# Cc19245/gaussian-splatting_CC-Comments

Hardware: AMD Instinct MI355X
Metric: train iters/sec (fwd+bwd rasterize) @1980x1080, 1M Gaussians (higher is better)
Workload: dtype f32; 1 GPU; C3: 1000000 Gaussians, SH deg 3, 1980x1080, mu=-5.0, seed 0; P=1000000, parallelism=single view

## Files before the change

gaussian-splatting_cc-comments_amd/csrc/api.hip:

```cpp
#include <stdarg.h>
#include <stdio.h>
#include <string.h>

#include <atomic>
#include <mutex>
#include <string>
#include <vector>

#include "gsr_internal.h"
#include "../../include/gsr_aa.h"

#define GSR_MAX_DEVICES 64
#ifndef GSR_COLOR_BESIDE_WGS
#define GSR_COLOR_BESIDE_WGS 2
#endif
#define GSR_COLOR_BESIDE_MAX_P 1500000

static thread_local char g_err[512] = "";

int gsr_fail(int code, const char* fmt, ...)
{
	va_list ap;
	va_start(ap, fmt);
	vsnprintf(g_err, sizeof g_err, fmt, ap);
	va_end(ap);
	return code;
}

int gsr_check_hip(hipError_t e, const char* what)
{
	if (e == hipSuccess) return GSR_OK;
	return gsr_fail(GSR_ERR_HIP, "%s: %s", what, hipGetErrorString(e));
}

int gsr_stage_done(hipStream_t s, int debug, const char* stage)
{
	hipError_t e = hipGetLastError();
	if (e != hipSuccess) return gsr_fail(GSR_ERR_HIP, "launch of %s failed: %s", stage, hipGetErrorString(e));
	if (debug & GSR_DEBUG_SYNC) {
		e = hipStreamSynchronize(s);
		if (e != hipSuccess) return gsr_fail(GSR_ERR_HIP, "[HIP ERROR] in stage %s: %s", stage, hipGetErrorString(e));
	}
	return GSR_OK;
}

extern "C" const char* gsr_last_error(void) { return g_err; }
extern "C" const char* gsr_version(void) { return "gsr-hip gfx950 r4"; }

struct ProfEntry { const char* name; hipEvent_t a, b; };
struct ProfRecorder {
	hipStream_t stream;
	bool on = false, open = false;
	std::vector<ProfEntry> ev;
	size_t used = 0;
	char only[64] = "";
};
static std::mutex g_prof_mu;
static std::vector<ProfRecorder*> g_prof;
static std::atomic<int> g_prof_active{0};

static ProfRecorder* prof_find(hipStream_t s, bool create)
{
	for (ProfRecorder* r : g_prof)
		if (r->stream == s) return r;
	if (!create) return nullptr;
	ProfRecorder* r = new ProfRecorder();
	r->stream = s;
	g_prof.push_back(r);
	return r;
}

static ProfEntry& prof_next(ProfRecorder* r, const char* name)
{
	if (r->used == r->ev.size()) {
		ProfEntry e;
		e.name = name;
		(void)hipEventCreate(&e.a);
		(void)hipEventCreate(&e.b);
		r->ev.push_back(e);
	}
	ProfEntry& e = r->ev[r->used++];
	e.name = name;
	return e;
}

bool gsr_prof_kernel_events(hipStream_t s, const char* name, hipEvent_t* a, hipEvent_t* b)
{
	if (g_prof_active.load(std::memory_order_relaxed) == 0) return false;
	std::lock_guard<std::mutex> lk(g_prof_mu);
	ProfRecorder* r = prof_find(s, false);
	if (!r || !r->on || !r->only[0] || strcmp(r->only, name) != 0) return false;
	ProfEntry& e = prof_next(r, name);
	r->open = false;
	*a = e.a;
	*b = e.b;
	return true;
}

void gsr_prof_mark_begin(hipStream_t s, const char* name)
{
	if (!name || g_prof_active.load(std::memory_order_relaxed) == 0) return;
	std::lock_guard<std::mutex> lk(g_prof_mu);
	ProfRecorder* r = prof_find(s, false);
	if (!r || !r->on) return;
	r->open = false;
	if (r->only[0] && strcmp(r->only, name) != 0) return;
	r->open = true;
	(void)hipEventRecord(prof_next(r, name).a, s);
}

void gsr_prof_mark_end(hipStream_t s)
{
	if (g_prof_active.load(std::memory_order_relaxed) == 0) return;
	std::lock_guard<std::mutex> lk(g_prof_mu);
	ProfRecorder* r = prof_find(s, false);
	if (!r || !r->on || !r->open || r->used == 0) return;
	r->open = false;
	(void)hipEventRecord(r->ev[r->used - 1].b, s);
}

static bool gsr_prof_records_all(hipStream_t s)
{
	if (g_prof_active.load(std::memory_order_relaxed) == 0) return false;
	std::lock_guard<std::mutex> lk(g_prof_mu);
	ProfRecorder* r = prof_find(s, false);
	return r && r->on && !r->only[0];
}

extern "C" int gsr_profile_begin_only(void* stream, const char* stage)
{
	std::lock_guard<std::mutex> lk(g_prof_mu);
	ProfRecorder* r = prof_find((hipStream_t)stream, true);
	if (!r->on) g_prof_active.fetch_add(1);
	r->on = true;
	r->open = false;
	r->used = 0;
	r->only[0] = 0;
	if (stage) { strncpy(r->only, stage, sizeof r->only - 1); r->only[sizeof r->only - 1] = 0; }
	return GSR_OK;
}

extern "C" int gsr_profile_begin(void* stream) { return gsr_profile_begin_only(stream, nullptr); }

extern "C" int gsr_profile_end(void* stream, gsr_kernel_time* out, int capacity)
{
	std::lock_guard<std::mutex> lk(g_prof_mu);
	ProfRecorder* r = prof_find((hipStream_t)stream, false);
	if (!r || !r->on) return 0;
	r->on = false;
	g_prof_active.fetch_sub(1);
	int n = 0;
	for (size_t k = 0; k < r->used; k++) {
		ProfEntry& e = r->ev[k];
		(void)hipEventSynchronize(e.b);
		float ms = 0.f;
		(void)hipEventElapsedTime(&ms, e.a, e.b);
		if (out && n < capacity) { out[n].name = e.name; out[n].ms = ms; n++; }
	}
	r->used = 0;
	return n;
}

extern "C" int gsr_geometry_layout_of(int P, gsr_geometry_layout* o)
{
	if (P < 0 || !o) return gsr_fail(GSR_ERR_INVALID_ARGUMENT, "gsr_geometry_layout_of: bad arguments");
	const size_t n = (size_t)P;
	const size_t nb = (n + GSR_PREPROCESS_BLOCK - 1) / GSR_PREPROCESS_BLOCK;
	size_t off = 0;
	o->splat = off;          off = gsr_align_up(off + n * sizeof(GsrSplat));
	o->depth_keys = off;     off = gsr_align_up(off + n * 4);
	o->depth_keys_alt = off; off = gsr_align_up(off + n * 4);
	o->perm = off;           off = gsr_align_up(off + n * 4);
	o->perm_alt = off;       off = gsr_align_up(off + n * 4);
	o->tiles_touched = off;  off = gsr_align_up(off + n * 4);
	o->rect = off;           off = gsr_align_up(off + n * 8);
	o->slot_base = off;      off = gsr_align_up(off + n * 4);
	o->clamped = off;        off = gsr_align_up(off + n);
	o->sh_ddir = off;        off = gsr_align_up(off + n * 36);
	o->status = off;         off = gsr_align_up(off + GSR_STATUS_WORDS * 4);
	o->scan_temp = off;      off = gsr_align_up(off + 2 * gsr_align_up(nb * 4));
	o->sort_table = off;     off = gsr_align_up(off + gsr_radix_table_bytes(n));
	o->col_table = off;      off = gsr_align_up(off + gsr_tilebin_col_table_bytes(n));
	o->rshape = off;         off = gsr_align_up(off + n * 8);
	o->total = off;
	return GSR_OK;
}

extern "C" int gsr_image_layout_of(int W, int H, gsr_image_layout* o)
{
	if (W < 0 || H < 0 || !o) return gsr_fail(GSR_ERR_INVALID_ARGUMENT, "gsr_image_layout_of: bad arguments");
	const size_t N = (size_t)W * H, T = (size_t)gsr_grid_x(W) * gsr_grid_y(H);
	size_t off = 0;
	o->final_C = off;          off = gsr_align_up(off + 3 * N * 4);
	o->final_T = off;          off = gsr_align_up(off + N * 4);
	o->n_contrib = off;        off = gsr_align_up(off + N * 4);
	o->ranges = off;           off = gsr_align_up(off + T * 8);
	o->tile_max_contrib = off; off = gsr_align_up(off + T * 4);
	{
		const size_t extra_f = 3 * (size_t)gsr_tile_order_max_split((int)T), extra_b = gsr_tile_order_max_segments((int)T);
		o->tile_order = off;   off = gsr_align_up(off + (T + (extra_f > extra_b ? extra_f : extra_b) + 1) * 4);
	}
	o->total = off;
	return GSR_OK;
}

extern "C" int gsr_binning_layout_of(int P, int64_t R, int W, int H, gsr_binning_layout* o)
{
	(void)P;
	if (R < 0 || W < 0 || H < 0 || !o) return gsr_fail(GSR_ERR_INVALID_ARGUMENT, "gsr_binning_layout_of: bad arguments");
	const size_t n = (size_t)R;
	size_t off = 0;
	o->point_list = off;     off = gsr_align_up(off + n * 4);
	o->point_list_alt = off; off = gsr_align_up(off + n * 4);
	o->tile_keys = off;      off = gsr_align_up(off + n * 4);
	o->tile_keys_alt = off;  off = gsr_align_up(off + n * 4);
	{
		const size_t a = gsr_radix_table_bytes(n), b = gsr_tilebin_row_table_bytes(n);
		o->sort_table = off; off = gsr_align_up(off + (a > b ? a : b));
	}
	o->checkpoints = off;    off = gsr_align_up(off + gsr_checkpoint_records(R) * 256 * sizeof(float4));
	o->total = off;
	o->tile_key_bytes = (size_t)gsr_tile_key_bytes(gsr_grid_x(W) * gsr_grid_y(H), n);
	o->column_pairs = gsr_tilebin_applies(W, H) ? 1 : 0;
	return GSR_OK;
}

extern "C" size_t gsr_geometry_bytes(int P)
{
	gsr_geometry_layout l;
	return gsr_geometry_layout_of(P, &l) == GSR_OK ? l.total : 0;
}
extern "C" size_t gsr_image_bytes(int W, int H)
{
	gsr_image_layout l;
	return gsr_image_layout_of(W, H, &l) == GSR_OK ? l.total : 0;
}
extern "C" size_t gsr_binning_bytes(int P, int64_t R, int W, int H)
{
	gsr_binning_layout l;
	return gsr_binning_layout_of(P, R, W, H, &l) == GSR_OK ? l.total : 0;
}
extern "C" size_t gsr_backward_scratch_bytes(int P, int64_t R)
{
	(void)P;
	if (R < 0) return 0;
	return gsr_align_up((size_t)R * sizeof(GsrGradSlot));
}

extern "C" int gsr_aux_layout_of(int64_t R, int W, int H, gsr_aux_layout* o)
{
	if (R < 0 || W < 0 || H < 0 || !o) return gsr_fail(GSR_ERR_INVALID_ARGUMENT, "gsr_aux_layout_of: bad arguments");
	size_t off = 0;
	o->ckpt_depth = off; off = gsr_align_up(off + gsr_checkpoint_records(R) * 256 * sizeof(float));
	o->final_D = off;    off = gsr_align_up(off + (size_t)W * H * sizeof(float));
	o->total = off;
	return GSR_OK;
}
extern "C" size_t gsr_aux_bytes(int64_t R, int W, int H)
{
	gsr_aux_layout l;
	return gsr_aux_layout_of(R, W, H, &l) == GSR_OK ? l.total : 0;
}
static const GsrAuxBlend* gsr_aux_view(const gsr_aux_args* x, int64_t R, int W, int H, GsrAuxBlend* a)
{
	if (!x) return nullptr;
	gsr_aux_layout l;
	gsr_aux_layout_of(R, W, H, &l);
	char* b = (char*)x->scratch;
	a->out_depth = x->out_depth; a->out_alpha = x->out_alpha;
	a->ckpt_depth = (float*)(b + l.ckpt_depth);
	a->final_D = (float*)(b + l.final_D);
	a->dL_ddepth = x->dL_ddepth; a->dL_dalpha = x->dL_dalpha;
	return a;
}

static bool aligned16(const void* p) { return ((uintptr_t)p & 15u) == 0; }

enum GsrAuxNeeds {
	GSR_AUX_NEEDS_MODE,
	GSR_AUX_NEEDS_SCRATCH,
	GSR_AUX_NEEDS_OUTPUTS
};
static int gsr_option_check(const char* who, int antialiasing, const gsr_aux_args* aux, bool optional, GsrAuxNeeds needs, bool live)
{
	if (antialiasing != 0 && antialiasing != 1) return gsr_fail(GSR_ERR_INVALID_ARGUMENT, "%s: antialiasing must be 0 or 1, got %d", who, antialiasing);
	if (!aux) return optional ? GSR_OK : gsr_fail(GSR_ERR_INVALID_ARGUMENT, "%s: aux is NULL", who);
	if (aux->mode != GSR_AUX_DEPTH && aux->mode != GSR_AUX_INVDEPTH) return gsr_fail(GSR_ERR_INVALID_ARGUMENT, "%s: the mode of aux is unknown", who);
	if (needs == GSR_AUX_NEEDS_MODE) return GSR_OK;
	if (!aligned16(aux->scratch)) return gsr_fail(GSR_ERR_INVALID_ARGUMENT, "%s: scratch must be 16-byte aligned", who);
	if (live && (!aux->scratch || (needs == GSR_AUX_NEEDS_OUTPUTS && (!aux->out_depth || !aux->out_alpha))))
		return gsr_fail(GSR_ERR_INVALID_ARGUMENT, "%s: %sscratch is NULL", who, needs == GSR_AUX_NEEDS_OUTPUTS ? "out_depth, out_alpha or " : "");
	return GSR_OK;
}

GsrGeometry gsr_geometry_view(void* blob, int P)
{
	gsr_geometry_layout l;
	gsr_geometry_layout_of(P, &l);
	char* b = (char*)blob;
	GsrGeometry g;
	g.splat = (GsrSplat*)(b + l.splat);
	g.depth_keys = (uint32_t*)(b + l.depth_keys);
	g.depth_keys_alt = (uint32_t*)(b + l.depth_keys_alt);
	g.perm = (uint32_t*)(b + l.perm);
	g.perm_alt = (uint32_t*)(b + l.perm_alt);
	g.tiles_touched = (uint32_t*)(b + l.tiles_touched);
	g.rect = (uint2*)(b + l.rect);
	g.slot_base = (uint32_t*)(b + l.slot_base);
	g.clamped = (uint8_t*)(b + l.clamped);
	g.sh_ddir = (float*)(b + l.sh_ddir);
	g.status = (uint32_t*)(b + l.status);
	g.sorted_block_sums = (uint32_t*)(b + l.scan_temp);
	g.block_tiles = (uint32_t*)(b + l.scan_temp + gsr_align_up(((size_t)P + GSR_PREPROCESS_BLOCK - 1) / GSR_PREPROCESS_BLOCK * 4));
	g.sort_table = (void*)(b + l.sort_table);
	g.col_table = (void*)(b + l.col_table);
	g.rshape = (uint2*)(b + l.rshape);
	return g;
}

GsrImage gsr_image_view(void* blob, int W, int H)
{
	gsr_image_layout l;
	gsr_image_layout_of(W, H, &l);
	char* b = (char*)blob;
	GsrImage im;
	im.final_C = (float*)(b + l.final_C);
	im.final_T = (float*)(b + l.final_T);
	im.n_contrib = (uint32_t*)(b + l.n_contrib);
	im.ranges = (uint2*)(b + l.ranges);
	im.tile_max_contrib = (uint32_t*)(b + l.tile_max_contrib);
	im.tile_order = (uint32_t*)(b + l.tile_order);
	return im;
}

GsrBinning gsr_binning_view(void* blob, int P, int64_t R, int W, int H)
{
	gsr_binning_layout l;
	gsr_binning_layout_of(P, R, W, H, &l);
	char* b = (char*)blob;
	GsrBinning bn;
	bn.point_list = (uint32_t*)(b + l.point_list);
	bn.point_list_alt = (uint32_t*)(b + l.point_list_alt);
	bn.tile_keys = (uint32_t*)(b + l.tile_keys);
	bn.tile_keys_alt = (uint32_t*)(b + l.tile_keys_alt);
	bn.sort_table = (void*)(b + l.sort_table);
	bn.checkpoints = (float4*)(b + l.checkpoints);
	return bn;
}

extern "C" uint32_t gsr_get_higher_msb(uint32_t n)
{
	uint32_t msb = sizeof(n) * 4;
	uint32_t step = msb;
	while (step > 1) {
		step /= 2;
		if (n >> msb) msb += step; else msb -= step;
	}
	if (n >> msb) msb++;
	return msb;
}

struct GsrThreadDevice {
	hipStream_t aux_stream = nullptr;
	hipEvent_t aux_fork = nullptr, aux_join = nullptr;
	uint32_t* status_host = nullptr;
	hipEvent_t status_event = nullptr;
	hipStream_t copy_stream = nullptr;
	hipEvent_t copy_fork = nullptr;
};
struct GsrThreadState { GsrThreadDevice dev[GSR_MAX_DEVICES]; };
static thread_local GsrThreadState g_thread;

extern "C" int gsr_thread_release(void)
{
	g_err[0] = 0;
	int rc = GSR_OK;
	for (int d = 0; d < GSR_MAX_DEVICES; d++) {
		GsrThreadDevice& t = g_thread.dev[d];
		if (t.aux_stream) { (void)hipStreamSynchronize(t.aux_stream); if (hipStreamDestroy(t.aux_stream) != hipSuccess) rc = GSR_ERR_HIP; }
		if (t.aux_fork && hipEventDestroy(t.aux_fork) != hipSuccess) rc = GSR_ERR_HIP;
		if (t.aux_join && hipEventDestroy(t.aux_join) != hipSuccess) rc = GSR_ERR_HIP;
		if (t.status_event && hipEventDestroy(t.status_event) != hipSuccess) rc = GSR_ERR_HIP;
		if (t.copy_stream) { (void)hipStreamSynchronize(t.copy_stream); if (hipStreamDestroy(t.copy_stream) != hipSuccess) rc = GSR_ERR_HIP; }
		if (t.copy_fork && hipEventDestroy(t.copy_fork) != hipSuccess) rc = GSR_ERR_HIP;
		if (t.status_host && hipHostFree(t.status_host) != hipSuccess) rc = GSR_ERR_HIP;
		t = GsrThreadDevice();
	}
	if (rc) { (void)hipGetLastError(); return gsr_fail(rc, "gsr_thread_release: a HIP resource could not be freed"); }
	return GSR_OK;
}

static bool gsr_helper_stream(hipStream_t* stream, hipEvent_t* e0, hipEvent_t* e1)
{
	if (*stream) return true;
	hipStream_t st = nullptr;
	hipEvent_t a = nullptr, b = nullptr;
	if (hipStreamCreateWithFlags(&st, hipStreamNonBlocking) == hipSuccess && hipEventCreateWithFlags(&a, hipEventDisableTiming) == hipSuccess &&
	    (!e1 || hipEventCreateWithFlags(&b, hipEventDisableTiming) == hipSuccess)) {
		*stream = st; *e0 = a;
		if (e1) *e1 = b;
		return true;
	}
	(void)hipGetLastError();
	if (st) (void)hipStreamDestroy(st);
	if (a) (void)hipEventDestroy(a);
	if (b) (void)hipEventDestroy(b);
	return false;
}

struct GsrJoinOnExit {
	hipStream_t s;
	hipEvent_t ev = nullptr;
	explicit GsrJoinOnExit(hipStream_t st) : s(st) {}
	void arm(hipEvent_t e) { ev = e; }
	int now()
	{
		if (!ev) return GSR_OK;
		hipEvent_t e = ev;
		ev = nullptr;
		if (hipStreamWaitEvent(s, e, 0) == hipSuccess) return GSR_OK;
		(void)hipEventSynchronize(e);
		return gsr_fail(GSR_ERR_HIP, "hipStreamWaitEvent(join) failed");
	}
	~GsrJoinOnExit()
	{
		if (ev && hipStreamWaitEvent(s, ev, 0) != hipSuccess) (void)hipEventSynchronize(ev);
	}
};

struct GsrDrainOnExit {
	hipStream_t st = nullptr;
	void arm(hipStream_t s) { st = s; }
	void disarm() { st = nullptr; }
	~GsrDrainOnExit() { if (st) (void)hipStreamSynchronize(st); }
};

struct GsrLastStage1 { const void* geometry = nullptr; bool col_pairs = false; };
static thread_local GsrLastStage1 g_last_stage1;

static int gsr_forward_preprocess_impl(const GsrPreprocessArgs& in, void* geometry, int64_t* num_rendered_host, void* stream, int debug,
                                       int aux, int aa)
{
	g_err[0] = 0;
	hipStream_t s = (hipStream_t)stream;
	GsrPreprocessArgs a = in;
	const int P = a.P, width = a.W, height = a.H;
	if (!num_rendered_host) return gsr_fail(GSR_ERR_INVALID_ARGUMENT, "num_rendered_host is NULL");
	*num_rendered_host = 0;
	if (P < 0 || width <= 0 || height <= 0) return gsr_fail(GSR_ERR_INVALID_ARGUMENT, "bad P / image size");
	if (P == 0) return GSR_OK;
	if (!a.means3D || !a.opacities || !a.viewmatrix || !a.projmatrix || !geometry)
		return gsr_fail(GSR_ERR_INVALID_ARGUMENT, "gsr_forward_preprocess: required pointer is NULL");
	if (!a.colors_precomp && !a.shs)
		return gsr_fail(GSR_ERR_INVALID_ARGUMENT, "For non-RGB, provide precomputed Gaussian colors!");
	if (!a.colors_precomp && (a.M <= 0 || (a.D + 1) * (a.D + 1) > a.M || a.D < 0 || a.D > 3 || !a.cam_pos))
		return gsr_fail(GSR_ERR_INVALID_ARGUMENT, "SH degree %d needs %d coefficients, M = %d", a.D, (a.D + 1) * (a.D + 1), a.M);
	if (!a.cov3D_precomp && (!a.scales || !a.rotations))
		return gsr_fail(GSR_ERR_INVALID_ARGUMENT, "provide scales+rotations or cov3D_precomp");
	if (width > 65535 * GSR_TILE_X || height > 65535 * GSR_TILE_Y)
		return gsr_fail(GSR_ERR_INVALID_ARGUMENT, "image too large for 16-bit tile coordinates");
	if (!aligned16(geometry)) return gsr_fail(GSR_ERR_INVALID_ARGUMENT, "geometry buffer must be 16-byte aligned");

	if (a.leaf && (a.M > 1 && !a.shs_rest)) return gsr_fail(GSR_ERR_INVALID_ARGUMENT, "leaf mode: features_rest is NULL");
	if (a.leaf && a.M > 16) return gsr_fail(GSR_ERR_INVALID_ARGUMENT, "leaf mode: at most 16 SH coefficients (degree 3), M = %d", a.M);
	a.focal_y = height / (2.0f * a.tan_fovy);
	a.focal_x = width / (2.0f * a.tan_fovx);
	a.g = gsr_geometry_view(geometry, P);

	int rc;
	int device = 0;
	if ((rc = gsr_check_hip(hipGetDevice(&device), "hipGetDevice"))) return rc;
	if (device < 0 || device >= GSR_MAX_DEVICES) return gsr_fail(GSR_ERR_INVALID_ARGUMENT, "device index %d not supported", device);
	GsrThreadDevice& td = g_thread.dev[device];
	const bool col_pairs = gsr_tilebin_applies(width, height) && !(debug & GSR_DEBUG_TILE_SORT);
	a.trim = (col_pairs && !(debug & GSR_DEBUG_NO_TRIM)) ? 1 : 0;
	const bool color = gsr_preprocess_needs_color(a);
#ifdef GSR_AB_FORCE_RADIX_DEPTH
	const bool bucket = false;
#else
	const bool bucket = gsr_bucket_sort_applies(P) && !(debug & GSR_DEBUG_RADIX_DEPTH);
#endif
	const bool beside = color && !(debug & (GSR_DEBUG_SYNC | GSR_DEBUG_SERIAL)) && !gsr_prof_records_all(s) &&
	                    gsr_helper_stream(&td.aux_stream, &td.aux_fork, &td.aux_join);
	GsrJoinOnExit join(s);
	gsr_launch_zero_status(a.g.status, s, beside ? td.aux_fork : nullptr);
	if (beside) {
		if ((rc = gsr_check_hip(hipStreamWaitEvent(td.aux_stream, td.aux_fork, 0), "hipStreamWaitEvent(fork)"))) return rc;
		gsr_launch_preprocess_color(a, td.aux_stream, P <= GSR_COLOR_BESIDE_MAX_P ? GSR_COLOR_BESIDE_WGS : 0, aux);
		if (hipEventRecord(td.aux_join, td.aux_stream) != hipSuccess) {
			(void)hipStreamSynchronize(td.aux_stream);
			return gsr_fail(GSR_ERR_HIP, "hipEventRecord(join) failed");
		}
		join.arm(td.aux_join);
	}
	const bool copy_beside = !(debug & (GSR_DEBUG_SYNC | GSR_DEBUG_SERIAL)) && !gsr_prof_records_all(s) &&
	                         gsr_helper_stream(&td.copy_stream, &td.copy_fork, nullptr);
	{
		GsrProfScope p(s, "preprocess");
		gsr_launch_preprocess(a, s, copy_beside ? td.copy_fork : nullptr, aux, aa);
	}
	if ((rc = gsr_stage_done(s, debug, "preprocess"))) return rc;
	if (color && !beside) {
		GsrProfScope p(s, "preprocess_color");
		gsr_launch_preprocess_color(a, s, 0, aux);
	}
	if ((rc = gsr_stage_done(s, debug, "preprocess_color"))) return rc;

	if (!td.status_host) {
		if ((rc = gsr_check_hip(hipHostMalloc((void**)&td.status_host, GSR_STATUS_WORDS * 4, hipHostMallocDefault), "hipHostMalloc"))) return rc;
	}
	if (!td.status_event) {
		if ((rc = gsr_check_hip(hipEventCreateWithFlags(&td.status_event, hipEventDisableTiming), "hipEventCreate"))) return rc;
	}
	uint32_t* status_host = td.status_host;
	hipEvent_t ev = td.status_event;
	if (copy_beside && (rc = gsr_check_hip(hipStreamWaitEvent(td.copy_stream, td.copy_fork, 0), "hipStreamWaitEvent(copy fork)"))) return rc;
	hipStream_t cs = copy_beside ? td.copy_stream : s;
	GsrDrainOnExit drain;
	if (copy_beside) drain.arm(td.copy_stream);
	if ((rc = gsr_check_hip(hipMemcpyAsync(status_host, a.g.status, GSR_STATUS_WORDS * 4, hipMemcpyDeviceToHost, cs), "hipMemcpyAsync(num_rendered)"))) return rc;
	if ((rc = gsr_check_hip(hipEventRecord(ev, cs), "hipEventRecord"))) return rc;
	const uint32_t* bias = a.g.status + GSR_STATUS_NEGMIN;
	{
		GsrProfScope p(s, "depth_sort");
		if (bucket) {
			gsr_launch_depth_bucket_sort(a.g, P, col_pairs ? gsr_tilebin_seg(a.g, P) : nullptr, s);
			if (col_pairs) gsr_launch_tilebin_col_hist(a.g, P, 0, s, true);
			else gsr_launch_sorted_block_sums(a.g, P, 0, s);
		} else {
			gsr_radix_sort_passes(a.g.depth_keys, a.g.perm, a.g.depth_keys_alt, a.g.perm_alt, (size_t)P, 32, 4, 0, 3, a.g.sort_table, bias, 4, s);
			if (col_pairs) gsr_launch_tilebin_col_hist(a.g, P, 1, s);
			else gsr_launch_sorted_block_sums(a.g, P, 1, s);
			gsr_launch_slot_base_finish(a.g.slot_base, a.g.block_tiles, a.g.status, (size_t)P, s);
		}
	}
	if ((rc = gsr_stage_done(s, debug, "depth_sort"))) return rc;
	if ((rc = gsr_check_hip(hipEventSynchronize(ev), "hipEventSynchronize(num_rendered)"))) return rc;
	drain.disarm();
	g_last_stage1.geometry = geometry;
	g_last_stage1.col_pairs = col_pairs;
	if (status_host[0] & 1u)
		return gsr_fail(GSR_ERR_PREFILTERED, "Point is filtered although prefiltered is set. This shouldn't happen!");
	int64_t total = 0;
	uint32_t negmin = 0, kmax = 0;
	for (int k = 0; k < GSR_COUNT_PARTS; k++) {
		total += (int64_t)status_host[4 + k];
		negmin = status_host[GSR_STATUS_NEGMIN + k] > negmin ? status_host[GSR_STATUS_NEGMIN + k] : negmin;
		kmax = status_host[GSR_STATUS_MAX + k] > kmax ? status_host[GSR_STATUS_MAX + k] : kmax;
	}
	*num_rendered_host = total;
	const uint32_t kmin = ~negmin;
	const uint32_t culled_value = kmax >= kmin ? (kmax - kmin) + 1u : 0u;
	const int fourth = !bucket && ((culled_value >> 24) != 0u || (kmax >= kmin && kmax - kmin == 0xFFFFFFFFu));
	if ((rc = join.now())) return rc;
	if (fourth) {
		GsrProfScope p(s, "depth_sort");
		gsr_radix_sort_passes(a.g.depth_keys, a.g.perm, a.g.depth_keys_alt, a.g.perm_alt, (size_t)P, 32, 4, 3, 1, a.g.sort_table, bias, 4, s);
		if (col_pairs) {
			if ((rc = gsr_check_hip(hipMemsetAsync(a.g.col_table, 0, gsr_tilebin_col_clear_words((size_t)P) * 4, s), "hipMemsetAsync(col_table)"))) return rc;
			gsr_launch_tilebin_col_hist(a.g, P, 0, s);
		} else {
			gsr_launch_sorted_block_sums(a.g, P, 0, s);
		}
	}
	return gsr_stage_done(s, debug, "depth_sort");
}

static GsrPreprocessArgs gsr_preprocess_inputs(int P, int D, int M, int width, int height, const float* means3D, const float* shs,
                                               const float* colors_precomp, const float* opacities, const float* scales,
                                               float scale_modifier, const float* rotations, const float* cov3D_precomp,
                                               const float* viewmatrix, const float* projmatrix, const float* cam_pos, float tan_fovx,
                                               float tan_fovy, int prefiltered, int* radii)
{
	GsrPreprocessArgs a = {};
	a.P = P; a.D = D; a.M = M; a.W = width; a.H = height;
	a.means3D = means3D; a.shs = shs; a.colors_precomp = colors_precomp; a.opacities = opacities;
	a.scales = scales; a.scale_modifier = scale_modifier; a.rotations = rotations; a.cov3D_precomp = cov3D_precomp;
	a.viewmatrix = viewmatrix; a.projmatrix = projmatrix; a.cam_pos = cam_pos;
	a.tan_fovx = tan_fovx; a.tan_fovy = tan_fovy;
	a.prefiltered = prefiltered;
	a.radii = radii;
	return a;
}
static GsrPreprocessArgs gsr_preprocess_leaves(int P, int D, int M, int width, int height, const float* xyz, const float* features_dc,
                                               const float* features_rest, const float* opacity_logits, const float* log_scales,
                                               float scale_modifier, const float* raw_rotations, const float* viewmatrix,
                                               const float* projmatrix, const float* cam_pos, float tan_fovx, float tan_fovy,
                                               int prefiltered, int* radii)
{
	GsrPreprocessArgs a = gsr_preprocess_inputs(P, D, M, width, height, xyz, features_dc, nullptr, opacity_logits, log_scales, scale_modifier,
	                                            raw_rotations, nullptr, viewmatrix, projmatrix, cam_pos, tan_fovx, tan_fovy, prefiltered, radii);
	a.leaf = 1; a.shs_rest = features_rest;
	return a;
}

extern "C" int gsr_forward_preprocess(int P, int D, int M, int width, int height, const float* means3D,
                                      const float* shs, const float* colors_precomp, const float* opacities,
                                      const float* scales, float scale_modifier, const float* rotations,
                                      const float* cov3D_precomp, const float* viewmatrix, const float* projmatrix,
                                      const float* cam_pos, float tan_fovx, float tan_fovy, int prefiltered,
                                      int* radii, void* geometry, int64_t* num_rendered_host, void* stream, int debug)
{
	const GsrPreprocessArgs a = gsr_preprocess_inputs(P, D, M, width, height, means3D, shs, colors_precomp, opacities, scales, scale_modifier, rotations,
	                                                    cov3D_precomp, viewmatrix, projmatrix, cam_pos, tan_fovx, tan_fovy, prefiltered, radii);
	return gsr_forward_preprocess_impl(a, geometry, num_rendered_host, stream, debug, 0, 0);
}

extern "C" int gsr_forward_preprocess_leaf(int P, int D, int M, int width, int height, const float* xyz,
                                           const float* features_dc, const float* features_rest,
                                           const float* opacity_logits, const float* log_scales, float scale_modifier,
                                           const float* raw_rotations, const float* viewmatrix, const float* projmatrix,
                                           const float* cam_pos, float tan_fovx, float tan_fovy, int prefiltered,
                                           int* radii, void* geometry, int64_t* num_rendered_host, void* stream,
                                           int debug)
{
	const GsrPreprocessArgs a = gsr_preprocess_leaves(P, D, M, width, height, xyz, features_dc, features_rest, opacity_logits, log_scales, scale_modifier,
	                                                    raw_rotations, viewmatrix, projmatrix, cam_pos, tan_fovx, tan_fovy, prefiltered, radii);
	return gsr_forward_preprocess_impl(a, geometry, num_rendered_host, stream, debug, 0, 0);
}

extern "C" int gsr_forward_preprocess_aux(const gsr_aux_args* aux, int P, int D, int M, int width, int height, const float* means3D,
                                          const float* shs, const float* colors_precomp, const float* opacities,
                                          const float* scales, float scale_modifier, const float* rotations,
                                          const float* cov3D_precomp, const float* viewmatrix, const float* projmatrix,
                                          const float* cam_pos, float tan_fovx, float tan_fovy, int prefiltered,
                                          int* radii, void* geometry, int64_t* num_rendered_host, void* stream, int debug)
{
	int rc;
	if ((rc = gsr_option_check("gsr_forward_preprocess_aux", 0, aux, false, GSR_AUX_NEEDS_MODE, false))) return rc;
	const GsrPreprocessArgs a = gsr_preprocess_inputs(P, D, M, width, height, means3D, shs, colors_precomp, opacities, scales, scale_modifier, rotations,
	                                                    cov3D_precomp, viewmatrix, projmatrix, cam_pos, tan_fovx, tan_fovy, prefiltered, radii);
	return gsr_forward_preprocess_impl(a, geometry, num_rendered_host, stream, debug, aux->mode, 0);
}

extern "C" int gsr_forward_preprocess_leaf_aux(const gsr_aux_args* aux, int P, int D, int M, int width, int height, const float* xyz,
                                               const float* features_dc, const float* features_rest,
                                               const float* opacity_logits, const float* log_scales, float scale_modifier,
                                               const float* raw_rotations, const float* viewmatrix, const float* projmatrix,
                                               const float* cam_pos, float tan_fovx, float tan_fovy, int prefiltered,
                                               int* radii, void* geometry, int64_t* num_rendered_host, void* stream,
                                               int debug)
{
	int rc;
	if ((rc = gsr_option_check("gsr_forward_preprocess_leaf_aux", 0, aux, false, GSR_AUX_NEEDS_MODE, false))) return rc;
	const GsrPreprocessArgs a = gsr_preprocess_leaves(P, D, M, width, height, xyz, features_dc, features_rest, opacity_logits, log_scales, scale_modifier,
	                                                    raw_rotations, viewmatrix, projmatrix, cam_pos, tan_fovx, tan_fovy, prefiltered, radii);
	return gsr_forward_preprocess_impl(a, geometry, num_rendered_host, stream, debug, aux->mode, 0);
}

extern "C" int gsr_forward_preprocess_aa(int antialiasing, const gsr_aux_args* aux, int P, int D, int M, int width, int height,
                                         const float* means3D, const float* shs, const float* colors_precomp, const float* opacities,
                                         const float* scales, float scale_modifier, const float* rotations,
                                         const float* cov3D_precomp, const float* viewmatrix, const float* projmatrix,
                                         const float* cam_pos, float tan_fovx, float tan_fovy, int prefiltered,
                                         int* radii, void* geometry, int64_t* num_rendered_host, void* stream, int debug)
{
	int rc;
	if ((rc = gsr_option_check("gsr_forward_preprocess_aa", antialiasing, aux, true, GSR_AUX_NEEDS_MODE, false))) return rc;
	const GsrPreprocessArgs a = gsr_preprocess_inputs(P, D, M, width, height, means3D, shs, colors_precomp, opacities, scales, scale_modifier, rotations,
	                                                    cov3D_precomp, viewmatrix, projmatrix, cam_pos, tan_fovx, tan_fovy, prefiltered, radii);
	return gsr_forward_preprocess_impl(a, geometry, num_rendered_host, stream, debug, aux ? aux->mode : 0, antialiasing);
}

extern "C" int gsr_forward_preprocess_leaf_aa(int antialiasing, const gsr_aux_args* aux, int P, int D, int M, int width, int height,
                                              const float* xyz, const float* features_dc, const float* features_rest,
                                              const float* opacity_logits, const float* log_scales, float scale_modifier,
                                              const float* raw_rotations, const float* viewmatrix, const float* projmatrix,
                                              const float* cam_pos, float tan_fovx, float tan_fovy, int prefiltered,
                                              int* radii, void* geometry, int64_t* num_rendered_host, void* stream,
                                              int debug)
{
	int rc;
	if ((rc = gsr_option_check("gsr_forward_preprocess_leaf_aa", antialiasing, aux, true, GSR_AUX_NEEDS_MODE, false))) return rc;
	const GsrPreprocessArgs a = gsr_preprocess_leaves(P, D, M, width, height, xyz, features_dc, features_rest, opacity_logits, log_scales, scale_modifier,
	                                                    raw_rotations, viewmatrix, projmatrix, cam_pos, tan_fovx, tan_fovy, prefiltered, radii);
	return gsr_forward_preprocess_impl(a, geometry, num_rendered_host, stream, debug, aux ? aux->mode : 0, antialiasing);
}

static int gsr_forward_render_impl(int P, int64_t R, int width, int height, const float* background,
                                   const int* radii, void* geometry, void* binning, void* image, float* out_color,
                                   void* stream, int debug, const gsr_aux_args* aux)
{
	g_err[0] = 0;
	hipStream_t s = (hipStream_t)stream;
	if (P < 0 || R < 0 || width <= 0 || height <= 0) return gsr_fail(GSR_ERR_INVALID_ARGUMENT, "bad sizes");
	if (P == 0) return GSR_OK;
	if (!background || !geometry || !image || !out_color || (R > 0 && !binning))
		return gsr_fail(GSR_ERR_INVALID_ARGUMENT, "gsr_forward_render: required pointer is NULL");
	if (!aligned16(geometry) || !aligned16(image) || !aligned16(binning))
		return gsr_fail(GSR_ERR_INVALID_ARGUMENT, "state buffers must be 16-byte aligned");
	if (R > 0xffffffffLL) return gsr_fail(GSR_ERR_INVALID_ARGUMENT, "num_rendered exceeds 32-bit offsets");
	if ((int64_t)gsr_grid_x(width) * gsr_grid_y(height) >= (1 << 28))
		return gsr_fail(GSR_ERR_INVALID_ARGUMENT, "image too large: more than 2^28 tiles");

	GsrGeometry g = gsr_geometry_view(geometry, P);
	GsrImage im = gsr_image_view(image, width, height);
	const int ntiles = gsr_grid_x(width) * gsr_grid_y(height);
	int rc;
	int key_bytes = 4;
	GsrBinning b;
	memset(&b, 0, sizeof b);
	const bool col_pairs = gsr_tilebin_applies(width, height) && !(debug & GSR_DEBUG_TILE_SORT);
	if (g_last_stage1.geometry == geometry && g_last_stage1.col_pairs != col_pairs)
		return gsr_fail(GSR_ERR_INVALID_ARGUMENT, "gsr_forward_render: GSR_DEBUG_TILE_SORT must be passed to both forward calls or to neither "
		                "(gsr_forward_preprocess on this thread prepared this geometry buffer for the other binning)");
	if (R > 0) b = gsr_binning_view(binning, P, R, width, height);
	if (R > 0 && col_pairs) {
		{
			GsrProfScope p(s, "col_scatter");
			gsr_launch_tilebin_col_scatter(g, P, b, R, s);
		}
		if ((rc = gsr_stage_done(s, debug, "col_scatter"))) return rc;
		{
			GsrProfScope p(s, "row_hist");
			gsr_launch_tilebin_row_hist(g, P, b, R, s);
		}
		if ((rc = gsr_stage_done(s, debug, "row_hist"))) return rc;
		{
			GsrProfScope p(s, "row_scatter");
			gsr_launch_tilebin_row_scatter(g, P, b, R, im.ranges, width, height, s);
		}
		if ((rc = gsr_stage_done(s, debug, "row_scatter"))) return rc;
	} else {
		if (R > 0) {
			const int bit = (int)gsr_get_higher_msb((uint32_t)ntiles);
			const bool even = gsr_radix_num_passes(bit) % 2 == 0;
			uint32_t *k0 = even ? b.tile_keys : b.tile_keys_alt, *v0 = even ? b.point_list : b.point_list_alt;
			uint32_t *k1 = even ? b.tile_keys_alt : b.tile_keys, *v1 = even ? b.point_list_alt : b.point_list;
			key_bytes = gsr_tile_key_bytes(ntiles, (size_t)R);
			{
				GsrProfScope p(s, "duplicate_keys");
				gsr_launch_duplicate_keys(g, P, width, k0, key_bytes, v0, (uint32_t*)b.sort_table, gsr_radix_clear_words((size_t)R), s);
			}
			if ((rc = gsr_stage_done(s, debug, "duplicate_keys"))) return rc;
			{
				GsrProfScope p(s, "sort");
				int in_first = 1;
				gsr_radix_sort_u32(k0, v0, k1, v1, (size_t)R, bit, b.sort_table, &in_first, 0, key_bytes, s);
			}
			if ((rc = gsr_stage_done(s, debug, "sort"))) return rc;
		}
		{
			GsrProfScope p(s, "tile_ranges");
			gsr_launch_tile_ranges(b.tile_keys, key_bytes, R, im.ranges, ntiles, b.tile_keys_alt, s);
		}
		if ((rc = gsr_stage_done(s, debug, "tile_ranges"))) return rc;
	}
	if (R > 0) {
		GsrProfScope p(s, "tile_order");
		gsr_launch_tile_order(im, ntiles, false, R, !(debug & GSR_DEBUG_NO_SPLIT), s, col_pairs);
	}
	if ((rc = gsr_stage_done(s, debug, "tile_order"))) return rc;
	{
		GsrProfScope p(s, "render_forward");
		GsrAuxBlend x;
		gsr_launch_render_forward(width, height, im, b.point_list, g.splat, b.checkpoints, background, out_color, R > 0, !(debug & GSR_DEBUG_NO_CULL), s,
		                          gsr_aux_view(aux, R, width, height, &x));
	}
	return gsr_stage_done(s, debug, "render_forward");
}

extern "C" int gsr_forward_render(int P, int64_t R, int width, int height, const float* background,
                                  const int* radii, void* geometry, void* binning, void* image, float* out_color,
                                  void* stream, int debug)
{
	return gsr_forward_render_impl(P, R, width, height, background, radii, geometry, binning, image, out_color, stream, debug, nullptr);
}

extern "C" int gsr_forward_render_aux(const gsr_aux_args* aux, int P, int64_t R, int width, int height, const float* background,
                                      const int* radii, void* geometry, void* binning, void* image, float* out_color,
                                      void* stream, int debug)
{
	int rc;
	if ((rc = gsr_option_check("gsr_forward_render_aux", 0, aux, false, GSR_AUX_NEEDS_OUTPUTS, P > 0))) return rc;
	return gsr_forward_render_impl(P, R, width, height, background, radii, geometry, binning, image, out_color, stream, debug, aux);
}

static int gsr_backward_check(const gsr_backward_args& a, const char* who)
{
	if (a.P < 0 || a.num_rendered < 0 || a.width <= 0 || a.height <= 0) return gsr_fail(GSR_ERR_INVALID_ARGUMENT, "%s: bad sizes", who);
	if (a.P == 0) return GSR_OK;
	if (!a.background || !a.means3D || !a.viewmatrix || !a.projmatrix || !a.geometry || !a.image || !a.dL_dpix ||
	    !a.dL_dmean2D || !a.dL_dopacity || !a.dL_dmean3D || !a.dL_dscale || !a.dL_drot || (a.num_rendered > 0 && (!a.binning || !a.scratch)))
		return gsr_fail(GSR_ERR_INVALID_ARGUMENT, "gsr_backward: required pointer is NULL");
	if (!a.leaf && ((a.colors_precomp && !a.dL_dcolor) || (a.cov3D_precomp && !a.dL_dcov3D) || (a.shs && !a.dL_dsh && !a.dL_dcolor)))
		return gsr_fail(GSR_ERR_INVALID_ARGUMENT, "gsr_backward: the gradient of a provided input is NULL");
	if (a.leaf) {
		if (!a.shs || !a.scales || !a.rotations || (a.M > 1 && !a.shs_rest))
			return gsr_fail(GSR_ERR_INVALID_ARGUMENT, "gsr_backward_leaf: a leaf tensor is NULL");
		if (a.M > 16) return gsr_fail(GSR_ERR_INVALID_ARGUMENT, "gsr_backward_leaf: at most 16 SH coefficients (degree 3), M = %d", a.M);
		if ((a.dL_dsh == nullptr) != (a.dL_dsh_rest == nullptr) && a.M > 1)
			return gsr_fail(GSR_ERR_INVALID_ARGUMENT, "gsr_backward_leaf: pass both feature gradients or neither");
		if (!a.dL_dsh && !a.dL_dcolor)
			return gsr_fail(GSR_ERR_INVALID_ARGUMENT, "gsr_backward_leaf: without feature gradients dL_dRGB is required");
	}
	if (a.stat_max_radii2D && !a.radii)
		return gsr_fail(GSR_ERR_INVALID_ARGUMENT, "gsr_backward: stat_max_radii2D needs radii");
	if (!aligned16(a.geometry) || !aligned16(a.image) || !aligned16(a.binning) || !aligned16(a.scratch))
		return gsr_fail(GSR_ERR_INVALID_ARGUMENT, "state buffers must be 16-byte aligned");
	return GSR_OK;
}

static uint8_t* gsr_slot_valid_of(const gsr_backward_args& a)
{
	if (a.num_rendered <= 0) return nullptr;
	return (uint8_t*)gsr_binning_view(a.binning, a.P, a.num_rendered, a.width, a.height).tile_keys_alt;
}

static int gsr_backward_blend_impl(const gsr_backward_args* args, const gsr_aux_args* aux)
{
	g_err[0] = 0;
	if (!args) return gsr_fail(GSR_ERR_INVALID_ARGUMENT, "gsr_backward_blend: args is NULL");
	const gsr_backward_args& a = *args;
	int rc;
	if ((rc = gsr_backward_check(a, "gsr_backward_blend"))) return rc;
	if (a.P == 0 || a.num_rendered == 0) return GSR_OK;
	hipStream_t s = (hipStream_t)a.stream;
	GsrGeometry g = gsr_geometry_view(a.geometry, a.P);
	GsrImage im = gsr_image_view(a.image, a.width, a.height);
	GsrBinning b = gsr_binning_view(a.binning, a.P, a.num_rendered, a.width, a.height);
	{
		GsrProfScope p(s, "tile_order");
		gsr_launch_tile_order(im, gsr_grid_x(a.width) * gsr_grid_y(a.height), true, a.num_rendered, !(a.debug & GSR_DEBUG_NO_SPLIT), s);
	}
	if ((rc = gsr_stage_done(s, a.debug, "tile_order"))) return rc;
	{
		hipEvent_t t0 = nullptr, t1 = nullptr;
		const bool own = gsr_prof_kernel_events(s, "render_backward", &t0, &t1);
		GsrProfScope p(s, own ? nullptr : "render_backward");
		GsrAuxBlend x;
		gsr_launch_render_backward(a.width, a.height, im, b.point_list, g.splat, b.checkpoints, g.slot_base, a.background, a.dL_dpix,
		                           (GsrGradSlot*)a.scratch, (uint8_t*)b.tile_keys_alt, !(a.debug & GSR_DEBUG_NO_CULL), s, t0, t1,
		                           gsr_aux_view(aux, a.num_rendered, a.width, a.height, &x));
	}
	return gsr_stage_done(s, a.debug, "render_backward");
}

extern "C" int gsr_backward_blend(const gsr_backward_args* args) { return gsr_backward_blend_impl(args, nullptr); }

extern "C" int gsr_backward_blend_aux(const gsr_backward_args* args, const gsr_aux_args* aux)
{
	int rc;
	if ((rc = gsr_option_check("gsr_backward_blend_aux", 0, aux, false, GSR_AUX_NEEDS_SCRATCH, args && args->P > 0 && args->num_rendered > 0))) return rc;
	return gsr_backward_blend_impl(args, aux);
}

static int gsr_backward_gaussians_impl(const gsr_backward_args* args, int first, int count, int out_row0, int aux, const float* aa_opacities)
{
	g_err[0] = 0;
	if (!args) return gsr_fail(GSR_ERR_INVALID_ARGUMENT, "gsr_backward_gaussians: args is NULL");
	const gsr_backward_args& b = *args;
	int rc;
	if ((rc = gsr_backward_check(b, "gsr_backward_gaussians"))) return rc;
	if (first < 0 || count < 0 || (int64_t)first + count > b.P || (first & 63) || (out_row0 != 0 && out_row0 != first))
		return gsr_fail(GSR_ERR_INVALID_ARGUMENT, "gsr_backward_gaussians: bad range [%d, %d + %d) of %d Gaussians (first must be a multiple "
		                "of 64, out_row0 must be 0 or first)", first, first, count, b.P);
	if (count == 0) return GSR_OK;
	hipStream_t s = (hipStream_t)b.stream;
	GsrGaussianBackwardArgs a = {};
	a.leaf = b.leaf; a.shs_rest = b.shs_rest; a.dL_dsh_rest = b.dL_dsh_rest;
	a.P = b.P; a.D = b.D; a.M = b.M; a.W = b.width; a.H = b.height;
	a.first = first; a.count = count; a.out_row0 = out_row0;
	a.means3D = b.means3D; a.shs = b.shs; a.colors_precomp = b.colors_precomp; a.scales = b.scales;
	a.scale_modifier = b.scale_modifier; a.rotations = b.rotations; a.cov3D_precomp = b.cov3D_precomp;
	a.viewmatrix = b.viewmatrix; a.projmatrix = b.projmatrix; a.cam_pos = b.cam_pos;
	a.tan_fovx = b.tan_fovx; a.tan_fovy = b.tan_fovy;
	a.focal_y = b.height / (2.0f * b.tan_fovy);
	a.focal_x = b.width / (2.0f * b.tan_fovx);
	a.radii = b.radii; a.g = gsr_geometry_view(b.geometry, b.P);
	a.slots = (const GsrGradSlot*)b.scratch; a.slot_valid = gsr_slot_valid_of(b);
	a.dL_dmean2D = b.dL_dmean2D; a.dL_dconic = b.dL_dconic; a.dL_dopacity = b.dL_dopacity; a.dL_dcolor = b.dL_dcolor;
	a.dL_dmean3D = b.dL_dmean3D; a.dL_dcov3D = b.dL_dcov3D; a.dL_dsh = b.dL_dsh; a.dL_dscale = b.dL_dscale; a.dL_drot = b.dL_drot;
	a.stat_xyz_gradient_accum = b.stat_xyz_gradient_accum; a.stat_denom = b.stat_denom; a.stat_max_radii2D = b.stat_max_radii2D;
	{
		GsrProfScope p(s, "gaussian_backward");
		gsr_launch_gaussian_backward(a, aa_opacities, s, aux);
	}
	return gsr_stage_done(s, b.debug, "gaussian_backward");
}

extern "C" int gsr_backward_gaussians(const gsr_backward_args* args, int first, int count, int out_row0)
{
	return gsr_backward_gaussians_impl(args, first, count, out_row0, 0, nullptr);
}

extern "C" int gsr_backward_gaussians_aux(const gsr_backward_args* args, const gsr_aux_args* aux, int first, int count, int out_row0)
{
	int rc;
	if ((rc = gsr_option_check("gsr_backward_gaussians_aux", 0, aux, false, GSR_AUX_NEEDS_SCRATCH, false))) return rc;
	return gsr_backward_gaussians_impl(args, first, count, out_row0, aux->mode, nullptr);
}

extern "C" int gsr_backward_gaussians_aa(const gsr_backward_args* args, int antialiasing, const float* opacities, const gsr_aux_args* aux,
                                         int first, int count, int out_row0)
{
	int rc;
	if ((rc = gsr_option_check("gsr_backward_gaussians_aa", antialiasing, aux, true, GSR_AUX_NEEDS_SCRATCH, false))) return rc;
	if (antialiasing && args && args->P > 0 && count > 0 && !opacities)
		return gsr_fail(GSR_ERR_INVALID_ARGUMENT, "gsr_backward_gaussians_aa: the opacity input is NULL");
	return gsr_backward_gaussians_impl(args, first, count, out_row0, aux ? aux->mode : 0, antialiasing ? opacities : nullptr);
}

static int gsr_backward_whole(const gsr_backward_args& a)
{
	int rc;
	if ((rc = gsr_backward_blend(&a))) return rc;
	return gsr_backward_gaussians(&a, 0, a.P, 0);
}

extern "C" int gsr_backward(int P, int D, int M, int64_t R, int width, int height, const float* background,
                            const float* means3D, const float* shs, const float* colors_precomp,
                            const float* scales, float scale_modifier, const float* rotations,
                            const float* cov3D_precomp, const float* viewmatrix, const float* projmatrix,
                            const float* cam_pos, float tan_fovx, float tan_fovy, const int* radii, void* geometry,
                            void* binning, void* image, void* scratch, const float* dL_dpix, float* dL_dmean2D,
                            float* dL_dconic, float* dL_dopacity, float* dL_dcolor, float* dL_dmean3D,
                            float* dL_dcov3D, float* dL_dsh, float* dL_dscale, float* dL_drot, void* stream,
                            int debug)
{
	gsr_backward_args a = {};
	a.P = P; a.D = D; a.M = M; a.num_rendered = R; a.width = width; a.height = height; a.leaf = 0;
	a.background = background; a.means3D = means3D; a.shs = shs; a.colors_precomp = colors_precomp; a.scales = scales;
	a.scale_modifier = scale_modifier; a.rotations = rotations; a.cov3D_precomp = cov3D_precomp; a.viewmatrix = viewmatrix;
	a.projmatrix = projmatrix; a.cam_pos = cam_pos; a.tan_fovx = tan_fovx; a.tan_fovy = tan_fovy; a.radii = radii;
	a.geometry = geometry; a.binning = binning; a.image = image; a.scratch = scratch; a.dL_dpix = dL_dpix;
	a.dL_dmean2D = dL_dmean2D; a.dL_dconic = dL_dconic; a.dL_dopacity = dL_dopacity; a.dL_dcolor = dL_dcolor;
	a.dL_dmean3D = dL_dmean3D; a.dL_dcov3D = dL_dcov3D; a.dL_dsh = dL_dsh; a.dL_dscale = dL_dscale; a.dL_drot = dL_drot;
	a.stream = stream; a.debug = debug;
	return gsr_backward_whole(a);
}

extern "C" int gsr_backward_leaf(int P, int D, int M, int64_t R, int width, int height, const float* background,
                                 const float* xyz, const float* features_dc, const float* features_rest,
                                 const float* log_scales, float scale_modifier, const float* raw_rotations,
                                 const float* viewmatrix, const float* projmatrix, const float* cam_pos, float tan_fovx,
                                 float tan_fovy, const int* radii, void* geometry, void* binning, void* image,
                                 void* scratch, const float* dL_dpix, float* dL_dmean2D, float* dL_dxyz,
                                 float* dL_dfeatures_dc, float* dL_dfeatures_rest, float* dL_dopacity_logits,
                                 float* dL_dlog_scales, float* dL_draw_rotations, float* dL_dRGB, void* stream, int debug)
{
	gsr_backward_args a = {};
	a.P = P; a.D = D; a.M = M; a.num_rendered = R; a.width = width; a.height = height; a.leaf = 1;
	a.background = background; a.means3D = xyz; a.shs = features_dc; a.shs_rest = features_rest; a.scales = log_scales;
	a.scale_modifier = scale_modifier; a.rotations = raw_rotations; a.viewmatrix = viewmatrix; a.projmatrix = projmatrix;
	a.cam_pos = cam_pos; a.tan_fovx = tan_fovx; a.tan_fovy = tan_fovy; a.radii = radii;
	a.geometry = geometry; a.binning = binning; a.image = image; a.scratch = scratch; a.dL_dpix = dL_dpix;
	a.dL_dmean2D = dL_dmean2D; a.dL_dopacity = dL_dopacity_logits; a.dL_dcolor = dL_dRGB; a.dL_dmean3D = dL_dxyz;
	a.dL_dsh = dL_dfeatures_dc; a.dL_dsh_rest = dL_dfeatures_rest; a.dL_dscale = dL_dlog_scales; a.dL_drot = dL_draw_rotations;
	a.stream = stream; a.debug = debug;
	return gsr_backward_whole(a);
}

extern "C" size_t gsr_loss_scratch_bytes(int C, int H, int W)
{
	if (C <= 0 || H <= 0 || W <= 0) return 0;
	size_t a, b;
	int n;
	return gsr_loss_scratch_layout(C, H, W, &a, &b, &n);
}

extern "C" int gsr_l1_ssim_loss(int C, int H, int W, const float* img, const float* gt, float lambda_dssim, float* loss_out,
                                float* dL_dimg, void* scratch, void* stream)
{
	g_err[0] = 0;
	if (C <= 0 || H <= 0 || W <= 0) return gsr_fail(GSR_ERR_INVALID_ARGUMENT, "gsr_l1_ssim_loss: bad image size");
	if (!img || !gt || !loss_out || !scratch) return gsr_fail(GSR_ERR_INVALID_ARGUMENT, "gsr_l1_ssim_loss: NULL pointer");
	gsr_launch_l1_ssim(C, H, W, img, gt, lambda_dssim, loss_out, dL_dimg, scratch, (hipStream_t)stream);
	return gsr_stage_done((hipStream_t)stream, 0, "l1_ssim_loss");
}

extern "C" size_t gsr_knn_scratch_bytes(int P) { return gsr_knn_scratch_size(P); }

extern "C" int gsr_knn_mean_dist2(int P, const float* points, float* mean_dist2, void* scratch, void* stream)
{
	g_err[0] = 0;
	if (P < 0) return gsr_fail(GSR_ERR_INVALID_ARGUMENT, "gsr_knn_mean_dist2: negative point count");
	if (P == 0) return GSR_OK;
	if (!points || !mean_dist2 || !scratch) return gsr_fail(GSR_ERR_INVALID_ARGUMENT, "gsr_knn_mean_dist2: required pointer is NULL");
	if (!aligned16(scratch)) return gsr_fail(GSR_ERR_INVALID_ARGUMENT, "gsr_knn_mean_dist2: scratch must be 16-byte aligned");
	gsr_launch_knn(P, points, mean_dist2, scratch, (hipStream_t)stream);
	return gsr_check_hip(hipGetLastError(), "knn kernels");
}

extern "C" int gsr_adam_step(int ngroups, const gsr_adam_group* groups, double beta1, double beta2, double eps,
                             const int* radii, void* stream)
{
	g_err[0] = 0;
	if (ngroups < 0 || ngroups > GSR_ADAM_MAX_GROUPS) return gsr_fail(GSR_ERR_INVALID_ARGUMENT, "gsr_adam_step: 0..%d groups", GSR_ADAM_MAX_GROUPS);
	if (ngroups == 0) return GSR_OK;
	if (!groups) return gsr_fail(GSR_ERR_INVALID_ARGUMENT, "gsr_adam_step: groups is NULL");
	for (int k = 0; k < ngroups; k++) {
		const gsr_adam_group& g = groups[k];
		if (g.numel < 0 || g.step < 1 || (g.numel > 0 && (!g.param || !g.grad || !g.exp_avg || !g.exp_avg_sq)))
			return gsr_fail(GSR_ERR_INVALID_ARGUMENT, "gsr_adam_step: group %d: NULL tensor, negative size or step < 1", k);
		if (g.numel > ((int64_t)1 << 41)) return gsr_fail(GSR_ERR_INVALID_ARGUMENT, "gsr_adam_step: group %d too large", k);
		if (radii && (g.row <= 0 || g.numel % g.row != 0))
			return gsr_fail(GSR_ERR_INVALID_ARGUMENT, "gsr_adam_step: group %d: numel is not a multiple of row", k);
	}
	int64_t total = 0;
	for (int k = 0; k < ngroups; k++) total += groups[k].numel;
	if (total == 0) return GSR_OK;
	hipStream_t s = (hipStream_t)stream;
	{
		GsrProfScope p(s, "adam");
		gsr_launch_adam(ngroups, groups, beta1, beta2, eps, radii, s);
	}
	return gsr_check_hip(hipGetLastError(), "gsr_adam_kernel launch");
}

extern "C" int gsr_sh_grad_from_views(int P, int D, int M, int V, const float* means3D, const float* cam_pos,
                                      const float* dL_dRGB, int64_t view_stride, float* dL_dsh, void* stream)
{
	g_err[0] = 0;
	if (P < 0 || V < 0 || D < 0 || D > 3 || M <= 0 || M > 16 || (D + 1) * (D + 1) > M)
		return gsr_fail(GSR_ERR_INVALID_ARGUMENT, "gsr_sh_grad_from_views: bad sizes (P %d, V %d, D %d, M %d)", P, V, D, M);
	if (P == 0) return GSR_OK;
	if (!means3D || !dL_dsh || (V > 0 && (!cam_pos || !dL_dRGB)))
		return gsr_fail(GSR_ERR_INVALID_ARGUMENT, "gsr_sh_grad_from_views: NULL pointer");
	if (view_stride == 0) view_stride = (int64_t)P * 3;
	if (view_stride < (int64_t)P * 3) return gsr_fail(GSR_ERR_INVALID_ARGUMENT, "gsr_sh_grad_from_views: view_stride < 3 * P");
	gsr_launch_sh_grad_from_views(P, D, M, V, means3D, cam_pos, dL_dRGB, view_stride, dL_dsh, (hipStream_t)stream);
	return gsr_stage_done((hipStream_t)stream, 0, "sh_grad_from_views");
}

extern "C" int gsr_mark_visible(int P, const float* means3D, const float* viewmatrix, const float* projmatrix,
                                uint8_t* present, void* stream)
{
	g_err[0] = 0;
	(void)projmatrix;
	if (P < 0) return gsr_fail(GSR_ERR_INVALID_ARGUMENT, "bad P");
	if (P == 0) return GSR_OK;
	if (!means3D || !viewmatrix || !present) return gsr_fail(GSR_ERR_INVALID_ARGUMENT, "gsr_mark_visible: NULL pointer");
	gsr_launch_mark_visible(P, means3D, viewmatrix, present, (hipStream_t)stream);
	return gsr_stage_done((hipStream_t)stream, 0, "mark_visible");
}
```

gaussian-splatting_cc-comments_amd/csrc/binning.hip:

```cpp
#include "gsr_internal.h"

__device__ __forceinline__ uint32_t gsr_wave_incl_scan(uint32_t v)
{
	const int lane = threadIdx.x & 63;
#pragma unroll
	for (int off = 1; off < 64; off <<= 1) {
		uint32_t n = __shfl_up(v, off, 64);
		if (lane >= off) v += n;
	}
	return v;
}

template <int BLOCK>
__device__ __forceinline__ uint32_t gsr_block_incl_scan(uint32_t v, uint32_t* total, uint32_t* lds )
{
	const int lane = threadIdx.x & 63, wave = threadIdx.x >> 6;
	uint32_t incl = gsr_wave_incl_scan(v);
	if (lane == 63) lds[wave] = incl;
	__syncthreads();
	uint32_t base = 0, tot = 0;
#pragma unroll
	for (int w = 0; w < BLOCK / 64; w++) {
		uint32_t s = lds[w];
		if (w < wave) base += s;
		tot += s;
	}
	__syncthreads();
	*total = tot;
	return incl + base;
}

__global__ void __launch_bounds__(GSR_PREPROCESS_BLOCK) gsr_sorted_block_sums_kernel(const uint32_t* __restrict__ perm,
                                                                                    const uint32_t* __restrict__ tiles_touched,
                                                                                    int P, uint32_t* __restrict__ sums,
                                                                                    uint32_t* __restrict__ status, uint32_t result_in_alt)
{
	__shared__ uint32_t lds[GSR_PREPROCESS_BLOCK / 64];
	const int i = blockIdx.x * GSR_PREPROCESS_BLOCK + threadIdx.x;
	if (i == 0) status[2] = result_in_alt;
	const uint32_t t = (i < P) ? tiles_touched[perm[i]] : 0u;
	uint32_t total;
	(void)gsr_block_incl_scan<GSR_PREPROCESS_BLOCK>(t, &total, lds);
	if (threadIdx.x == 0) sums[blockIdx.x] = total;
}

void gsr_launch_sorted_block_sums(GsrGeometry g, int P, int result_in_alt, hipStream_t s)
{
	const int nb = (P + GSR_PREPROCESS_BLOCK - 1) / GSR_PREPROCESS_BLOCK;
	hipLaunchKernelGGL(gsr_sorted_block_sums_kernel, dim3(nb), dim3(GSR_PREPROCESS_BLOCK), 0, s, result_in_alt ? g.perm_alt : g.perm,
	                   g.tiles_touched, P, g.sorted_block_sums, g.status, (uint32_t)result_in_alt);
}

__global__ void __launch_bounds__(GSR_PREPROCESS_BLOCK) gsr_duplicate_keys_kernel(GsrGeometry g, int P, uint32_t gx,
                                                                                 void* __restrict__ keys_, int key_bytes,
                                                                                 uint32_t* __restrict__ vals,
                                                                                 uint32_t* __restrict__ clear, size_t clear_words)
{
	for (size_t w = (size_t)blockIdx.x * GSR_PREPROCESS_BLOCK + threadIdx.x; w < clear_words; w += (size_t)gridDim.x * GSR_PREPROCESS_BLOCK)
		clear[w] = 0u;
	const uint32_t* __restrict__ perm = g.status[2] ? g.perm_alt : g.perm;
	uint32_t* __restrict__ const keys32 = static_cast<uint32_t*>(keys_);
	uint16_t* __restrict__ const keys16 = static_cast<uint16_t*>(keys_);
	__shared__ uint32_t lds[GSR_PREPROCESS_BLOCK / 64];
	__shared__ uint4 s_own[GSR_PREPROCESS_BLOCK / 64][64];
	__shared__ uint32_t s_flag[GSR_PREPROCESS_BLOCK / 64][64];
	const int i = blockIdx.x * GSR_PREPROCESS_BLOCK + threadIdx.x;
	const int lane = threadIdx.x & 63, wave = threadIdx.x >> 6;
	uint32_t idx = 0, tiles = 0, rmin = 0, w = 1;
	if (i < P) {
		idx = perm[i];
		const uint2 rc = g.rect[idx];
		rmin = rc.x;
		w = rc.y & 0xffffu;
		tiles = w * (rc.y >> 16);
		if (!tiles) w = 1;
	}
	uint32_t before = 0;
	{
		const uint32_t* __restrict__ sums = g.sorted_block_sums;
		for (uint32_t b0 = 0; b0 < blockIdx.x; b0 += 8 * GSR_PREPROCESS_BLOCK) {
			uint32_t t[8];
#pragma unroll
			for (int j = 0; j < 8; j++) {
				const uint32_t b = b0 + j * GSR_PREPROCESS_BLOCK + threadIdx.x;
				t[j] = b < blockIdx.x ? sums[b] : 0u;
			}
#pragma unroll
			for (int j = 0; j < 8; j++) before += t[j];
		}
	}
	uint32_t total, before_total;
	(void)gsr_block_incl_scan<GSR_PREPROCESS_BLOCK>(before, &before_total, lds);
	const uint32_t incl = gsr_block_incl_scan<GSR_PREPROCESS_BLOCK>(tiles, &total, lds) + before_total;
	const uint32_t off = incl - tiles;
	const uint32_t wave_first = __shfl(off, 0, 64);
	const uint32_t wave_total = __shfl(incl, 63, 64) - wave_first;
	s_own[wave][lane] = make_uint4(off - wave_first, rmin, w, idx);
	__builtin_amdgcn_wave_barrier();
	const uint32_t mystart = off - wave_first;
	uint32_t carry = 0u;
	for (uint32_t j0 = 0; j0 < wave_total; j0 += 64) {
		s_flag[wave][lane] = 0u;
		__builtin_amdgcn_wave_barrier();
		const uint32_t rel = mystart - j0;
		if (tiles && rel < 64u) s_flag[wave][rel] = (uint32_t)lane + 1u;
		__builtin_amdgcn_wave_barrier();
		uint32_t o = s_flag[wave][lane];
		o = max(o, (uint32_t)__builtin_amdgcn_update_dpp(0, (int)o, 0x111, 0xF, 0xF, false));
		o = max(o, (uint32_t)__builtin_amdgcn_update_dpp(0, (int)o, 0x112, 0xF, 0xF, false));
		o = max(o, (uint32_t)__builtin_amdgcn_update_dpp(0, (int)o, 0x114, 0xF, 0xF, false));
		o = max(o, (uint32_t)__builtin_amdgcn_update_dpp(0, (int)o, 0x118, 0xF, 0xF, false));
		o = max(o, (uint32_t)__builtin_amdgcn_update_dpp(0, (int)o, 0x142, 0xA, 0xF, false));
		o = max(o, (uint32_t)__builtin_amdgcn_update_dpp(0, (int)o, 0x143, 0xC, 0xF, false));
		o = max(o, carry);
		carry = (uint32_t)__builtin_amdgcn_readlane((int)o, 63);
		__builtin_amdgcn_wave_barrier();
		const uint32_t j = j0 + lane;
		if (j >= wave_total) continue;
		const uint32_t lo = o - 1u;
		const uint4 own = s_own[wave][lo];
		const uint32_t k = j - own.x;
		const uint32_t rm = own.y, ww = own.z;
		uint32_t q;
		if (k < (1u << 22)) {
			q = (uint32_t)((float)k * __builtin_amdgcn_rcpf((float)ww));
			const int32_t r = (int32_t)(k - q * ww);
			q = r < 0 ? q - 1u : (r >= (int32_t)ww ? q + 1u : q);
		} else {
			q = k / ww;
		}
		const uint32_t y = (rm >> 16) + q, x = (rm & 0xffffu) + (k - q * ww);
		if (key_bytes == 2) keys16[wave_first + j] = (uint16_t)(y * gx + x);
		else keys32[wave_first + j] = y * gx + x;
		vals[wave_first + j] = own.w;
	}
}

void gsr_launch_duplicate_keys(GsrGeometry g, int P, int W, void* keys, int key_bytes, uint32_t* vals, uint32_t* clear, size_t clear_words, hipStream_t s)
{
	const int nb = (P + GSR_PREPROCESS_BLOCK - 1) / GSR_PREPROCESS_BLOCK;
	hipLaunchKernelGGL(gsr_duplicate_keys_kernel, dim3(nb), dim3(GSR_PREPROCESS_BLOCK), 0, s, g, P, (uint32_t)gsr_grid_x(W),
	                   keys, key_bytes, vals, clear, clear_words);
}

template <typename KeyT>
__global__ void __launch_bounds__(256) gsr_tile_ranges_kernel(const KeyT* __restrict__ tile_keys, int64_t L, uint2* ranges,
                                                              uint32_t ntiles, uint32_t* __restrict__ valid)
{
	const int64_t i0 = ((int64_t)blockIdx.x * 256 + threadIdx.x) * 4;
	if (i0 >= L) return;
	valid[i0 >> 2] = 0u;
	uint32_t k[4];
	if (i0 + 3 < L) {
		if constexpr (sizeof(KeyT) == 4) {
			const uint4 v = *reinterpret_cast<const uint4*>(tile_keys + i0);
			k[0] = v.x; k[1] = v.y; k[2] = v.z; k[3] = v.w;
		} else {
			const uint2 v = *reinterpret_cast<const uint2*>(tile_keys + i0);
			k[0] = v.x & 0xffffu; k[1] = v.x >> 16; k[2] = v.y & 0xffffu; k[3] = v.y >> 16;
		}
	} else {
#pragma unroll
		for (int j = 0; j < 4; j++) k[j] = (i0 + j < L) ? tile_keys[i0 + j] : 0u;
	}
	uint32_t prevtile = (i0 > 0) ? tile_keys[i0 - 1] : 0u;
#pragma unroll
	for (int j = 0; j < 4; j++) {
		const int64_t idx = i0 + j;
		if (idx >= L) break;
		const uint32_t currtile = k[j];
		if (idx == 0) {
			for (uint32_t t = 0; t < currtile; t++) ranges[t] = make_uint2(0u, 0u);
			ranges[currtile].x = 0;
		} else if (currtile != prevtile) {
			ranges[prevtile].y = (uint32_t)idx;
			for (uint32_t t = prevtile + 1; t < currtile; t++) ranges[t] = make_uint2(0u, 0u);
			ranges[currtile].x = (uint32_t)idx;
		}
		if (idx == L - 1) {
			ranges[currtile].y = (uint32_t)L;
			for (uint32_t t = currtile + 1; t < ntiles; t++) ranges[t] = make_uint2(0u, 0u);
		}
		prevtile = currtile;
	}
}

#define GSR_ORDER_BINS 1024
#define GSR_ORDER_PER_THREAD 9
__device__ __forceinline__ uint32_t gsr_tile_work(const uint2* ranges, const uint32_t* tile_max_contrib, uint32_t t)
{
#ifdef GSR_TILE_CLOCK
	if (!ranges) return tile_max_contrib[t];
#endif
	const uint2 r = ranges[t];
	uint32_t work = r.y - r.x;
	if (tile_max_contrib) work = min(work, tile_max_contrib[t]);
	return work;
}
__device__ __forceinline__ uint32_t gsr_tile_work_bin(uint32_t work)
{
	return GSR_ORDER_BINS - 1 - min(work >> 4, (uint32_t)GSR_ORDER_BINS - 1);
}

__device__ __forceinline__ uint32_t gsr_tile_segments(uint32_t work, uint32_t coarse)
{
	if (work < (coarse + 1u) * GSR_CKPT_STRIDE) return 1u;
	const uint32_t nblk = (work + GSR_CKPT_STRIDE - 1) / GSR_CKPT_STRIDE;
	const uint32_t m = (nblk + GSR_CKPT_MAX_SEGMENTS - 1) / GSR_CKPT_MAX_SEGMENTS * coarse;
	return (nblk + m - 1) / m;
}

#ifdef GSR_TILE_CLOCK
static uint32_t* g_debug_backward_key = nullptr;
extern "C" int gsr_debug_backward_key(uint32_t* key) { g_debug_backward_key = key; return 0; }
static uint32_t* g_debug_forward_key = nullptr;
extern "C" int gsr_debug_forward_key(uint32_t* key) { g_debug_forward_key = key; return 0; }
#endif

__global__ void __launch_bounds__(1024) gsr_tile_order_kernel(const uint2* ranges, const uint32_t* __restrict__ tile_max_contrib,
                                                              uint32_t ntiles, uint32_t* __restrict__ order, uint32_t split_min, uint32_t max_split,
                                                              uint32_t* tile_max_contrib_out, uint32_t seg_budget, int allow_cut,
                                                              uint2* ranges_fix)
{
	__shared__ uint32_t bin[GSR_ORDER_BINS];
	__shared__ uint32_t wsum[1024 / 64];
	__shared__ uint32_t s_nsplit, s_seg_items[4], s_seg_cursor, s_incl[GSR_ORDER_BINS], s_total;
	if (threadIdx.x == 0) { s_nsplit = 0u; s_seg_cursor = 0u; s_total = 0u; }
	if (threadIdx.x < 4) s_seg_items[threadIdx.x] = 0u;
	bin[threadIdx.x] = 0;
	uint32_t b0[GSR_ORDER_PER_THREAD], w0[GSR_ORDER_PER_THREAD];
#pragma unroll
	for (int j = 0; j < GSR_ORDER_PER_THREAD; j++) {
		const uint32_t t = j * 1024 + threadIdx.x;
		w0[j] = t < ntiles ? gsr_tile_work(ranges, tile_max_contrib, t) : 0u;
		b0[j] = t < ntiles ? gsr_tile_work_bin(w0[j]) : 0xffffffffu;
		if (ranges_fix && t < ntiles && w0[j] == 0u) ranges_fix[t] = make_uint2(0u, 0u);
	}
	if (ranges_fix)
		for (uint32_t t = 1024 * GSR_ORDER_PER_THREAD + threadIdx.x; t < ntiles; t += 1024) {
			const uint2 r = ranges_fix[t];
			if (r.x == r.y) ranges_fix[t] = make_uint2(0u, 0u);
		}
	__syncthreads();
	if (seg_budget && allow_cut) {
		uint32_t my_items[4] = {0u, 0u, 0u, 0u};
		auto count = [&](uint32_t w) {
			if (w < 2 * GSR_CKPT_STRIDE) return;
#pragma unroll
			for (int f = 0; f < 4; f++)
				if (w >= ((1u << f) + 1u) * GSR_CKPT_STRIDE) my_items[f] += gsr_tile_segments(w, 1u << f);
		};
#pragma unroll
		for (int j = 0; j < GSR_ORDER_PER_THREAD; j++) count(w0[j]);
		for (uint32_t t = 1024 * GSR_ORDER_PER_THREAD + threadIdx.x; t < ntiles; t += 1024) count(gsr_tile_work(ranges, tile_max_contrib, t));
#pragma unroll
		for (int f = 0; f < 4; f++)
			if (my_items[f]) atomicAdd(&s_seg_items[f], my_items[f]);
	}
	uint32_t my_work = 0u;
#pragma unroll
	for (int j = 0; j < GSR_ORDER_PER_THREAD; j++)
		if (b0[j] != 0xffffffffu) { atomicAdd(&bin[b0[j]], 1u); my_work += w0[j]; }
	for (uint32_t base = 1024 * GSR_ORDER_PER_THREAD; base < ntiles; base += 1024 * GSR_ORDER_PER_THREAD) {
		uint32_t b[GSR_ORDER_PER_THREAD];
#pragma unroll
		for (int j = 0; j < GSR_ORDER_PER_THREAD; j++) {
			const uint32_t t = base + j * 1024 + threadIdx.x;
			const uint32_t w = t < ntiles ? gsr_tile_work(ranges, tile_max_contrib, t) : 0u;
			b[j] = t < ntiles ? gsr_tile_work_bin(w) : 0xffffffffu;
			my_work += w;
		}
#pragma unroll
		for (int j = 0; j < GSR_ORDER_PER_THREAD; j++)
			if (b[j] != 0xffffffffu) atomicAdd(&bin[b[j]], 1u);
	}
	if (split_min) {
#pragma unroll
		for (int off = 32; off > 0; off >>= 1) my_work += (uint32_t)__shfl_xor((int)my_work, off, 64);
		if ((threadIdx.x & 63) == 0 && my_work) atomicAdd(&s_total, my_work);
	}
	__syncthreads();
	int split_bin_max = -1;
	if (split_min) {
		const uint32_t heavy = max(split_min, 2u * (s_total / max(ntiles, 1u)));
		split_bin_max = GSR_ORDER_BINS - 1 - (int)min((heavy + 15u) / 16u, (uint32_t)GSR_ORDER_BINS - 1u);
	}
	const uint32_t c = bin[threadIdx.x];
	uint32_t total;
	const uint32_t incl = gsr_block_incl_scan<1024>(c, &total, wsum);
	bin[threadIdx.x] = incl - c;
	if ((int)threadIdx.x <= split_bin_max && c != 0u && incl <= max_split) atomicMax(&s_nsplit, incl);
	s_incl[threadIdx.x] = incl;
	__syncthreads();
	uint32_t coarse = 0u, nheavy = 0u, front = 0u;
	if (seg_budget && allow_cut)
		for (int f = 0; f < 4 && !coarse; f++) {
			const uint32_t tiles_f = s_incl[GSR_ORDER_BINS - 1 - ((1u << f) + 1u) * (GSR_CKPT_STRIDE / 16)];
			if (s_seg_items[f] != 0u && s_seg_items[f] - tiles_f <= seg_budget) { coarse = 1u << f; nheavy = tiles_f; front = s_seg_items[f]; }
		}
	if (seg_budget && threadIdx.x == 0) order[ntiles + seg_budget] = coarse;
	const uint32_t nsplit = s_nsplit;
	auto place = [&](uint32_t q, uint32_t t) {
		if (q < nheavy) {
			const uint32_t ns = gsr_tile_segments(gsr_tile_work(ranges, tile_max_contrib, t), coarse);
			const uint32_t at = atomicAdd(&s_seg_cursor, ns);
			for (uint32_t k = 0; k < ns; k++) order[at + k] = t | ((k + 1u) << 28);
		} else if (nheavy) {
			order[front + (q - nheavy)] = t;
		} else if (q < nsplit) {
#pragma unroll
			for (uint32_t k = 0; k < 4; k++) order[4 * q + k] = t | ((k + 1u) << 28);
			tile_max_contrib_out[t] = 0u;
		} else {
			order[3 * nsplit + q] = t;
		}
	};
	if (max_split)
		for (uint32_t e = ntiles + 3 * nsplit + threadIdx.x; e < ntiles + 3 * max_split; e += 1024) order[e] = 0xFFFFFFFFu;
	if (seg_budget)
		for (uint32_t e = ntiles + (front - nheavy) + threadIdx.x; e < ntiles + seg_budget; e += 1024) order[e] = 0xFFFFFFFFu;
#pragma unroll
	for (int j = 0; j < GSR_ORDER_PER_THREAD; j++)
		if (b0[j] != 0xffffffffu) place(atomicAdd(&bin[b0[j]], 1u), j * 1024 + threadIdx.x);
	for (uint32_t base = 1024 * GSR_ORDER_PER_THREAD; base < ntiles; base += 1024 * GSR_ORDER_PER_THREAD) {
		uint32_t b[GSR_ORDER_PER_THREAD];
#pragma unroll
		for (int j = 0; j < GSR_ORDER_PER_THREAD; j++) {
			const uint32_t t = base + j * 1024 + threadIdx.x;
			b[j] = t < ntiles ? gsr_tile_work_bin(gsr_tile_work(ranges, tile_max_contrib, t)) : 0xffffffffu;
		}
#pragma unroll
		for (int j = 0; j < GSR_ORDER_PER_THREAD; j++)
			if (b[j] != 0xffffffffu) place(atomicAdd(&bin[b[j]], 1u), base + j * 1024 + threadIdx.x);
	}
}

uint32_t gsr_tile_order_max_segments(int ntiles) { return (uint32_t)(ntiles < 64 ? 0 : (ntiles / 2 < 4096 ? ntiles / 2 : 4096)); }
uint32_t gsr_tile_order_max_split(int ntiles) { return (uint32_t)(ntiles < 64 ? 0 : (ntiles / 4 < 2048 ? ntiles / 4 : 2048)); }

void gsr_launch_tile_order(GsrImage img, int ntiles, bool backward, int64_t num_rendered, bool split, hipStream_t s, bool normalise_empty)
{
	const uint32_t* key = backward ? img.tile_max_contrib : (const uint32_t*)nullptr;
	const uint2* ranges = img.ranges;
#ifdef GSR_TILE_CLOCK
	if (backward && g_debug_backward_key) { key = g_debug_backward_key; ranges = nullptr; }
	if (!backward && g_debug_forward_key) { key = g_debug_forward_key; ranges = nullptr; split = false; }
#endif
	(void)num_rendered;
	const uint32_t max_split = backward ? 0u : gsr_tile_order_max_split(ntiles);
	const uint32_t split_min = (!backward && split && max_split) ? (uint32_t)GSR_SPLIT_MIN_LIST : 0u;
	const uint32_t seg_budget = backward ? gsr_tile_order_max_segments(ntiles) : 0u;
	int allow_cut = split ? 1 : 0;
#ifdef GSR_TILE_CLOCK
	if (!ranges) allow_cut = 0;
#endif
	hipLaunchKernelGGL(gsr_tile_order_kernel, dim3(1), dim3(1024), 0, s, ranges, key, (uint32_t)ntiles, img.tile_order, split_min, max_split,
	                   img.tile_max_contrib, seg_budget, allow_cut, (normalise_empty && !backward) ? img.ranges : (uint2*)nullptr);
}

void gsr_launch_tile_ranges(const void* tile_keys, int key_bytes, int64_t R, uint2* ranges, int ntiles, uint32_t* valid, hipStream_t s)
{
	if (R > 0 && key_bytes == 2)
		hipLaunchKernelGGL(gsr_tile_ranges_kernel<uint16_t>, dim3((unsigned)((R + 1023) / 1024)), dim3(256), 0, s, (const uint16_t*)tile_keys, R,
		                   ranges, (uint32_t)ntiles, valid);
	else if (R > 0)
		hipLaunchKernelGGL(gsr_tile_ranges_kernel<uint32_t>, dim3((unsigned)((R + 1023) / 1024)), dim3(256), 0, s, (const uint32_t*)tile_keys, R,
		                   ranges, (uint32_t)ntiles, valid);
	else
		(void)hipMemsetAsync(ranges, 0, (size_t)ntiles * sizeof(uint2), s);
}
```

gaussian-splatting_cc-comments_amd/csrc/gsr_internal.h:

```cpp
#pragma once
#include <hip/hip_runtime.h>
#include <hip/hip_ext.h>
#include <stddef.h>
#include <stdint.h>

#include <type_traits>

#include "../../include/gsr.h"
#include "../../include/gsr_aux.h"
#include "gsr_device.h"

#define GSR_PREPROCESS_BLOCK 256
#define GSR_COUNT_PARTS 64
#define GSR_STATUS_NEGMIN (4 + GSR_COUNT_PARTS)
#define GSR_STATUS_MAX (4 + 2 * GSR_COUNT_PARTS)
#define GSR_STATUS_WORDS (4 + 3 * GSR_COUNT_PARTS)

static inline size_t gsr_align_up(size_t v, size_t a = 256) { return (v + a - 1) / a * a; }
static inline int gsr_grid_x(int W) { return (W + GSR_TILE_X - 1) / GSR_TILE_X; }
static inline int gsr_grid_y(int H) { return (H + GSR_TILE_Y - 1) / GSR_TILE_Y; }

struct GsrGeometry {
	GsrSplat* splat;
	uint32_t* depth_keys;
	uint32_t* depth_keys_alt;
	uint32_t* perm;
	uint32_t* perm_alt;
	uint32_t* tiles_touched;
	uint2* rect;
	uint2* rshape;
	uint32_t* slot_base;
	uint8_t* clamped;
	float* sh_ddir;
	uint32_t* status;

	uint32_t* sorted_block_sums;
	uint32_t* block_tiles;
	void* sort_table;
	void* col_table;
};

#ifndef GSR_CKPT_STRIDE
#define GSR_CKPT_STRIDE 512
#endif
#ifndef GSR_SPLIT_MIN_LIST
#define GSR_SPLIT_MIN_LIST 640
#endif
#define GSR_CKPT_MAX_SEGMENTS 15
static inline size_t gsr_checkpoint_records(int64_t R) { return (size_t)(R / GSR_CKPT_STRIDE) + 2; }

struct GsrImage {
	float* final_C;
	float* final_T;
	uint32_t* n_contrib;
	uint2* ranges;
	uint32_t* tile_max_contrib;
	uint32_t* tile_order;
};

struct GsrBinning {
	uint32_t* point_list;
	uint32_t* point_list_alt;
	uint32_t* tile_keys;
	uint32_t* tile_keys_alt;
	void* sort_table;
	float4* checkpoints;
};

struct GsrAuxBlend {
	float* out_depth;
	float* out_alpha;
	float* ckpt_depth;
	float* final_D;
	const float* dL_ddepth;
	const float* dL_dalpha;
};

GsrGeometry gsr_geometry_view(void* blob, int P);
GsrImage gsr_image_view(void* blob, int W, int H);
GsrBinning gsr_binning_view(void* blob, int P, int64_t R, int W, int H);

int gsr_fail(int code, const char* fmt, ...);
int gsr_check_hip(hipError_t e, const char* what);
int gsr_stage_done(hipStream_t s, int debug, const char* stage);
void gsr_prof_mark_begin(hipStream_t s, const char* name);
void gsr_prof_mark_end(hipStream_t s);
bool gsr_prof_kernel_events(hipStream_t s, const char* name, hipEvent_t* a, hipEvent_t* b);

struct GsrProfScope {
	hipStream_t s;
	GsrProfScope(hipStream_t st, const char* name) : s(st) { gsr_prof_mark_begin(s, name); }
	~GsrProfScope() { gsr_prof_mark_end(s); }
};

template <typename T> struct GsrSame { typedef T type; };
template <typename... P>
static inline void gsr_launch(void (*kernel)(P...), dim3 grid, dim3 block, size_t lds, hipStream_t s, hipEvent_t start, hipEvent_t stop,
                              typename GsrSame<P>::type... args)
{
	if (start || stop) hipExtLaunchKernelGGL(kernel, grid, block, lds, s, start, stop, 0, args...);
	else hipLaunchKernelGGL(kernel, grid, block, lds, s, args...);
}

template <typename F>
static inline void gsr_variant(bool leaf, int aux, bool aa, F&& f)
{
	auto with_leaf = [&](auto AUX, auto AA) {
		if (leaf) f(std::true_type{}, AUX, AA);
		else f(std::false_type{}, AUX, AA);
	};
	auto with_aux = [&](auto AA) {
		if (aux == GSR_AUX_INVDEPTH) with_leaf(std::integral_constant<int, GSR_AUX_INVDEPTH>{}, AA);
		else if (aux) with_leaf(std::integral_constant<int, GSR_AUX_DEPTH>{}, AA);
		else with_leaf(std::integral_constant<int, 0>{}, AA);
	};
	if (aa) with_aux(std::true_type{});
	else with_aux(std::false_type{});
}

struct GsrPreprocessArgs {
	int P, D, M, W, H;
	const float* means3D;
	const float* shs;
	const float* colors_precomp;
	const float* opacities;
	const float* scales;
	float scale_modifier;
	const float* rotations;
	const float* cov3D_precomp;
	const float* viewmatrix;
	const float* projmatrix;
	const float* cam_pos;
	float tan_fovx, tan_fovy, focal_x, focal_y;
	int prefiltered;
	int trim;
	int* radii;
	GsrGeometry g;
	int leaf;
	const float* shs_rest;
};

void gsr_launch_preprocess(const GsrPreprocessArgs& a, hipStream_t s, hipEvent_t done, int aux, int aa);
void gsr_launch_zero_status(uint32_t* status, hipStream_t s, hipEvent_t done);
bool gsr_preprocess_needs_color(const GsrPreprocessArgs& a);
void gsr_launch_preprocess_color(const GsrPreprocessArgs& a, hipStream_t s, int wgs_per_cu, int aux);
void gsr_launch_mark_visible(int P, const float* means3D, const float* viewmatrix, uint8_t* present, hipStream_t s);

void gsr_launch_sorted_block_sums(GsrGeometry g, int P, int result_in_alt, hipStream_t s);
void gsr_launch_duplicate_keys(GsrGeometry g, int P, int W, void* keys, int key_bytes, uint32_t* vals, uint32_t* clear, size_t clear_words, hipStream_t s);
void gsr_launch_tile_ranges(const void* tile_keys, int key_bytes, int64_t R, uint2* ranges, int ntiles, uint32_t* valid, hipStream_t s);
void gsr_launch_tile_order(GsrImage img, int ntiles, bool backward, int64_t num_rendered, bool split, hipStream_t s, bool normalise_empty = false);
uint32_t gsr_tile_order_max_split(int ntiles);
uint32_t gsr_tile_order_max_segments(int ntiles);

bool gsr_tilebin_applies(int W, int H);
size_t gsr_tilebin_col_clear_words(size_t P);
size_t gsr_tilebin_col_table_bytes(size_t P);
size_t gsr_tilebin_row_clear_words(size_t R);
size_t gsr_tilebin_row_table_bytes(size_t R);
void gsr_launch_tilebin_col_hist(GsrGeometry g, int P, int result_in_alt, hipStream_t s, bool seg_ready = false);
uint4* gsr_tilebin_seg(GsrGeometry g, int P);
uint4* gsr_tilebin_recs(GsrGeometry g, int P);
void gsr_launch_tilebin_col_scatter(GsrGeometry g, int P, GsrBinning b, int64_t R, hipStream_t s);
void gsr_launch_tilebin_row_hist(GsrGeometry g, int P, GsrBinning b, int64_t R, hipStream_t s);
void gsr_launch_tilebin_row_scatter(GsrGeometry g, int P, GsrBinning b, int64_t R, uint2* ranges, int W, int H, hipStream_t s);

int gsr_radix_num_passes(int nbits_total);
size_t gsr_radix_table_bytes(size_t n);
size_t gsr_radix_clear_words(size_t n);
void gsr_launch_slot_base_finish(uint32_t* slot_base, const uint32_t* block_tiles, uint32_t* status, size_t n, hipStream_t s);
void gsr_radix_sort_passes(void* k0, uint32_t* v0, void* k1, uint32_t* v1, size_t n, int nbits_total, int npass_total,
                           int pass_first, int pass_count, void* table_mem, const uint32_t* bias, int key_bytes, hipStream_t s);
void gsr_radix_sort_u32(void* k0, uint32_t* v0, void* k1, uint32_t* v1, size_t n, int nbits_total, void* table_mem,
                        int* result_in_first, int clear_table, int key_bytes, hipStream_t s);
void gsr_radix_top_pass(const uint32_t* k0, uint32_t* k1, const uint2* rec_in, uint4* rec_out, size_t n, void* table_mem, const uint32_t* bias, hipStream_t s,
                        uint32_t* slot_base, const uint32_t* block_tiles, uint32_t* status);
int gsr_radix_top_chunks(size_t n);
#ifndef GSR_BUCKET_SORT_MAX_P
#define GSR_BUCKET_SORT_MAX_P (2 << 20)
#endif
bool gsr_bucket_sort_applies(int P);
void gsr_launch_depth_bucket_sort(GsrGeometry g, int P, uint4* seg, hipStream_t s);
int gsr_tile_key_bytes(int ntiles, size_t num_rendered);

void gsr_launch_render_forward(int W, int H, GsrImage img, const uint32_t* point_list, const GsrSplat* splat, float4* checkpoints,
                               const float* bg, float* out_color, bool ordered, bool cull, hipStream_t s,
                               const GsrAuxBlend* aux);

void gsr_launch_render_backward(int W, int H, GsrImage img, const uint32_t* point_list, const GsrSplat* splat, const float4* checkpoints,
                                const uint32_t* slot_base, const float* bg, const float* dL_dpix, GsrGradSlot* slots,
                                uint8_t* slot_valid, bool cull, hipStream_t s, hipEvent_t t_start, hipEvent_t t_stop,
                                const GsrAuxBlend* aux);

struct GsrGaussianBackwardArgs {
	int P, D, M, W, H;
	int first, count;
	int out_row0;
	const float* means3D;
	const float* shs;
	const float* colors_precomp;
	const float* scales;
	float scale_modifier;
	const float* rotations;
	const float* cov3D_precomp;
	const float* viewmatrix;
	const float* projmatrix;
	const float* cam_pos;
	float tan_fovx, tan_fovy, focal_x, focal_y;
	const int* radii;
	GsrGeometry g;
	const GsrGradSlot* slots;
	const uint8_t* slot_valid;
	float* dL_dmean2D;
	float* dL_dconic;
	float* dL_dopacity;
	float* dL_dcolor;
	float* dL_dmean3D;
	float* dL_dcov3D;
	float* dL_dsh;
	float* dL_dscale;
	float* dL_drot;
	int leaf;
	const float* shs_rest;
	float* dL_dsh_rest;
	float* stat_xyz_gradient_accum;
	float* stat_denom;
	float* stat_max_radii2D;
};
struct GsrGaussianBackwardArgsAA : GsrGaussianBackwardArgs {
	const float* opacities;
};
void gsr_launch_gaussian_backward(const GsrGaussianBackwardArgs& a, const float* aa_opacities, hipStream_t s, int aux);
void gsr_launch_sh_grad_from_views(int P, int D, int M, int V, const float* means3D, const float* cam_pos, const float* dL_dRGB,
                                   int64_t view_stride, float* dL_dsh, hipStream_t s);

size_t gsr_loss_scratch_layout(int C, int H, int W, size_t* maps_off, size_t* partial_off, int* ntiles);
void gsr_launch_l1_ssim(int C, int H, int W, const float* img, const float* gt, float lambda, float* loss_out, float* dL_dimg,
                        void* scratch, hipStream_t s);

int gsr_launch_adam(int ngroups, const gsr_adam_group* groups, double beta1, double beta2, double eps, const int* radii, hipStream_t s);

size_t gsr_knn_scratch_size(int P);
void gsr_launch_knn(int P, const float* points, float* mean_dist2, void* scratch, hipStream_t s);
```

gaussian-splatting_cc-comments_amd/csrc/render_backward.hip:

```cpp
#include "render_common.h"

#define GSR_BWD_NV 9
#define GSR_BWD_FLUSH 4
typedef float v2f __attribute__((ext_vector_type(2)));

GSR_TILE_CLOCK_BUFFER(gsr_backward_tile_clock, gsr_debug_tile_clock_backward)

__device__ __forceinline__ float gsr_add_halves(v2f a)
{
	float r;
	asm("v_add_f32_e32 %0, %1, %2" : "=v"(r) : "v"(a.x), "v"(a.y));
	return r;
}

template <bool AUX>
__global__ void __launch_bounds__(64 * GSR_WAVES_PER_WG) __attribute__((amdgpu_waves_per_eu(4, 4))) gsr_render_backward_wave_kernel(
	int W, int H, int gx, int nslots, const uint2* __restrict__ ranges, const uint32_t* __restrict__ point_list,
	const GsrSplat* __restrict__ splat, const float4* __restrict__ checkpoints, const float* __restrict__ final_C, const uint32_t* __restrict__ slot_base, const float* __restrict__ bg,
	const float* __restrict__ final_Ts, const uint32_t* __restrict__ n_contrib, const uint32_t* __restrict__ tile_max_contrib,
	const uint32_t* __restrict__ tile_order, const float* __restrict__ dL_dpixels, GsrGradSlot* __restrict__ slots,
	uint8_t* __restrict__ slot_valid, int cull, GsrAuxBlend aux)
{
	__shared__ float4 s_rec[GSR_WAVES_PER_WG][AUX ? 6 : 5][64];
	__shared__ uint32_t s_bands[GSR_WAVES_PER_WG][64];
	__shared__ float s_red[GSR_WAVES_PER_WG][64 * 9 + 8];
	__shared__ __attribute__((aligned(16))) float s_pend[GSR_WAVES_PER_WG][AUX ? 4 : GSR_BWD_FLUSH * 128];
	const int wave = threadIdx.x >> 6, lane = threadIdx.x & 63;
	const int slot_id = blockIdx.x * GSR_WAVES_PER_WG + wave;
	if (slot_id >= nslots) return;
	GSR_TILE_CLOCK_START();
	GSR_TILE_STAT(unsigned long long st_staged = 0; unsigned long long st_pairs = 0; unsigned long long st_pairs_hit = 0; unsigned long long st_reductions = 0; unsigned long long st_lanes_hit = 0;)
	const uint32_t entry = __builtin_amdgcn_readfirstlane(tile_order[slot_id]);
	if (entry == 0xFFFFFFFFu) return;
	const int tile = (int)(entry & 0x0FFFFFFFu);
	const int seg1 = (int)(entry >> 28);
	float4(*rec)[64] = s_rec[wave];
	uint32_t* recb = s_bands[wave];

	const int tx = tile % gx, ty = tile / gx;
	const int px = tx * GSR_TILE_X + (lane & 15);
	const int py0 = ty * GSR_TILE_Y + (lane >> 4);
	const v2f pfx2 = {(float)px, (float)px};
	const float x0f = (float)(tx * GSR_TILE_X), y0f = (float)(ty * GSR_TILE_Y);

	const uint2 range = ranges[tile];
	const int n = (int)min(range.y - range.x, tile_max_contrib[tile]);
	int seg_a = 0, top = n;
	if (seg1) {
		const int coarse = (int)__builtin_amdgcn_readfirstlane(tile_order[nslots]);
		const int nblk = (n + GSR_CKPT_STRIDE - 1) / GSR_CKPT_STRIDE, m = (nblk + GSR_CKPT_MAX_SEGMENTS - 1) / GSR_CKPT_MAX_SEGMENTS * coarse;
		seg_a = (seg1 - 1) * m * GSR_CKPT_STRIDE;
		top = min(n, seg1 * m * GSR_CKPT_STRIDE);
	}
	const int nw = top - seg_a;
	const uint32_t* plist = point_list + range.x;
	const size_t plane = (size_t)H * W;
	const float bg0 = bg[0], bg1 = bg[1], bg2 = bg[2];
	const float ddelx_dx = 0.5f * W, ddely_dy = 0.5f * H;

	v2f T[2], tfb[2];
	v2f ac0[2], ac1[2], ac2[2];
	v2f dp0[2], dp1[2], dp2[2];
	v2f dpD[2], acD[2];
	int last_contributor[GSR_PIX_PER_LANE];
	v2f pfy[2];
#pragma unroll
	for (int k = 0; k < GSR_PIX_PER_LANE; k++) {
		const int py = py0 + 4 * k;
		const bool inside = px < W && py < H;
		const uint32_t pix_id = inside ? (uint32_t)(W * py + px) : 0u;
		const float Tf = inside ? final_Ts[pix_id] : 0.f;
		const float d0 = inside ? dL_dpixels[pix_id] : 0.f;
		const float d1 = inside ? dL_dpixels[plane + pix_id] : 0.f;
		const float d2 = inside ? dL_dpixels[2 * plane + pix_id] : 0.f;
		last_contributor[k] = inside ? (int)n_contrib[pix_id] : 0;
		T[k >> 1][k & 1] = Tf;
		dp0[k >> 1][k & 1] = d0; dp1[k >> 1][k & 1] = d1; dp2[k >> 1][k & 1] = d2;
		if (AUX) {
			const float dD = (inside && aux.dL_ddepth) ? aux.dL_ddepth[pix_id] : 0.f;
			const float dA = (inside && aux.dL_dalpha) ? aux.dL_dalpha[pix_id] : 0.f;
			dpD[k >> 1][k & 1] = dD;
			tfb[k >> 1][k & 1] = -Tf * ((bg0 * d0 + bg1 * d1 + bg2 * d2) - dA);
		} else {
			tfb[k >> 1][k & 1] = -Tf * (bg0 * d0 + bg1 * d1 + bg2 * d2);
		}
		pfy[k >> 1][k & 1] = (float)py;
	}
#pragma unroll
	for (int p = 0; p < 2; p++) {
		ac0[p] = ac1[p] = ac2[p] = v2f{0.f, 0.f};
		if (AUX) acD[p] = v2f{0.f, 0.f};
	}
	if (top < n) {
		const float4* ck = checkpoints + ((size_t)(range.x + (uint32_t)top) / GSR_CKPT_STRIDE) * 256 + lane;
#pragma unroll
		for (int k = 0; k < GSR_PIX_PER_LANE; k++) {
			const int py = py0 + 4 * k;
			const bool inside = px < W && py < H;
			const uint32_t pix_id = inside ? (uint32_t)(W * py + px) : 0u;
			if (inside && last_contributor[k] > top) {
				const float4 c = ck[64 * k];
				const float inv = 1.0f / c.x;
				T[k >> 1][k & 1] = c.x;
				ac0[k >> 1][k & 1] = (final_C[pix_id] - c.y) * inv;
				ac1[k >> 1][k & 1] = (final_C[plane + pix_id] - c.z) * inv;
				ac2[k >> 1][k & 1] = (final_C[2 * plane + pix_id] - c.w) * inv;
				if (AUX) acD[k >> 1][k & 1] = (aux.final_D[pix_id] - aux.ckpt_depth[((size_t)(range.x + (uint32_t)top) / GSR_CKPT_STRIDE) * 256 + lane + 64 * k]) * inv;
			}
		}
	}
	int pair_last[2];
#pragma unroll
	for (int p = 0; p < 2; p++) {
		int m = max(last_contributor[2 * p], last_contributor[2 * p + 1]);
#pragma unroll
		for (int off = 32; off > 0; off >>= 1) m = max(m, __shfl_xor(m, off, 64));
		pair_last[p] = __builtin_amdgcn_readfirstlane(m);
	}

	float4 ra = make_float4(0, 0, 0, 0), rb = ra, rc = ra;
	uint32_t sbase = 0u;
	if (lane < nw) {
		const uint32_t id = plist[top - 1 - lane];
		const float4* p = reinterpret_cast<const float4*>(splat + id);
		ra = p[0]; rb = p[1]; rc = p[2];
		sbase = slot_base[id];
	}
	uint32_t id_next = (64 + lane < nw) ? plist[top - 1 - (64 + lane)] : 0u;
	const int out_index = lane >> 3;
	float* const red_w = s_red[wave] + lane * 9;
	const float* const red_r = s_red[wave] + (lane & 7) * 9 + (lane >> 3);
	constexpr int red_step = 72;
	const float out_scale = (out_index >= 2 && out_index <= 4) ? -0.5f : 1.0f;
	const float k01 = out_index == 0 ? -ddelx_dx : -ddely_dy;
	const int f_inst = (lane >> 3) & 3, f_val = lane & 7;
	float* const pend_w = s_pend[wave] + lane;
	const float* const pend_r = s_pend[wave] + f_inst * 128 + (lane >> 5) * 64 + f_val * 8;
	const float f_scale = (f_val >= 2 && f_val <= 4) ? -0.5f : 1.0f;
	const float f_k01 = f_val == 0 ? -ddelx_dx : -ddely_dy;
	const bool f_word = lane < 32 || f_val == 0;
	int npend = 0;
	uint32_t pend_j = 0u;

	for (int base = 0; base < nw; base += 64) {
		const uint32_t bands = (base + lane < nw) ? (cull ? gsr_tile_band_mask(ra.x, ra.y, ra.z, ra.w, rb.x, rb.y, x0f, y0f) : 0xFu) : 0u;
		const bool keep = bands != 0u;
		const unsigned long long mask = __builtin_amdgcn_ballot_w64(keep);
		const int cnt = __popcll(mask);
		GSR_TILE_STAT(st_staged += (unsigned)cnt;)
		if (keep) {
			const int pos = gsr_mbcnt(mask);
			const uint32_t rmin = __float_as_uint(rb.z), rwh = __float_as_uint(rb.w);
			const uint32_t slot = sbase + ((uint32_t)ty - (rmin >> 16)) * (rwh & 0xffffu) + ((uint32_t)tx - (rmin & 0xffffu));
			rec[0][pos] = make_float4(ra.x, ra.x, ra.y, ra.y);
			rec[1][pos] = make_float4(-0.5f * ra.z, -0.5f * ra.z, ra.w, ra.w);
			rec[2][pos] = make_float4(-0.5f * rb.x, -0.5f * rb.x, rb.y, rb.y);
			rec[3][pos] = make_float4(rc.x, rc.x, rc.y, rc.y);
			rec[4][pos] = make_float4(rc.z, rc.z, __int_as_float(top - 1 - (base + lane)), __uint_as_float(slot));
			if (AUX) rec[5][pos] = make_float4(rc.w, rc.w, 0.f, 0.f);
			recb[pos] = bands;
		}
		if (base + 64 + lane < nw) {
			const float4* p = reinterpret_cast<const float4*>(splat + id_next);
			ra = p[0]; rb = p[1]; rc = p[2];
			sbase = slot_base[id_next];
		}
		id_next = (base + 128 + lane < nw) ? plist[top - 1 - (base + 128 + lane)] : 0u;
		__builtin_amdgcn_wave_barrier();

#pragma clang loop unroll(disable)
		for (int j = 0; j < cnt; j++) {
			const float4 R0 = rec[0][j], R1 = rec[1][j], R2 = rec[2][j], R3 = rec[3][j], R4 = rec[4][j];
			const int contributor = __builtin_amdgcn_readfirstlane(__float_as_int(R4.z));
			const uint32_t bands = __builtin_amdgcn_readfirstlane(recb[j]);
			const v2f X = {R0.x, R0.y}, Y = {R0.z, R0.w}, CA = {R1.x, R1.y}, CB = {R1.z, R1.w}, CC = {R2.x, R2.y}, OP = {R2.z, R2.w};
			const v2f C0 = {R3.x, R3.y}, C1 = {R3.z, R3.w}, C2 = {R4.x, R4.y};
			v2f V = {0.f, 0.f};
			if (AUX) { const float4 R5 = rec[5][j]; V = v2f{R5.x, R5.y}; }
			const v2f dx = X - pfx2;
			const v2f ax2 = (CA * dx) * dx, bdx = CB * dx;
			v2f acc[GSR_BWD_NV + 1];
#pragma unroll
			for (int i = 0; i < GSR_BWD_NV + 1; i++) acc[i] = v2f{-0.f, -0.f};
			unsigned long long any = 0ull;
#pragma unroll
			for (int p = 0; p < 2; p++) {
				if (!(bands & (3u << (2 * p))) || contributor >= pair_last[p]) continue;
				const v2f dy = Y - pfy[p];
				const v2f power = (ax2 + (CC * dy) * dy) - bdx * dy;
				const v2f pl = power * 1.44269504088896340736f;
				const v2f G = {__builtin_amdgcn_exp2f(pl.x), __builtin_amdgcn_exp2f(pl.y)};
				const v2f og = OP * G;
				const v2f araw = {fminf(0.99f, og.x), fminf(0.99f, og.y)};
				const bool c0 = contributor < last_contributor[2 * p], p0 = !(power.x > 0.0f), a0 = !(araw.x < 1.0f / 255.0f);
				const bool c1 = contributor < last_contributor[2 * p + 1], p1 = !(power.y > 0.0f), a1 = !(araw.y < 1.0f / 255.0f);
				const bool hit0 = c0 && p0 && a0, hit1 = c1 && p1 && a1;
				const unsigned long long hits = (__builtin_amdgcn_ballot_w64(c0) & __builtin_amdgcn_ballot_w64(p0) & __builtin_amdgcn_ballot_w64(a0)) |
				                                (__builtin_amdgcn_ballot_w64(c1) & __builtin_amdgcn_ballot_w64(p1) & __builtin_amdgcn_ballot_w64(a1));
				GSR_TILE_STAT(st_pairs++;)
				if (hits == 0ull) continue;
				GSR_TILE_STAT(st_pairs_hit++; st_lanes_hit += (unsigned)__popcll(hits);)
				any |= hits;
				const v2f alpha = {hit0 ? araw.x : 0.f, hit1 ? araw.y : 0.f};
				const v2f oma = 1.f - alpha;
				const v2f inv1ma = {__builtin_amdgcn_rcpf(oma.x), __builtin_amdgcn_rcpf(oma.y)};
				const v2f Tn = T[p] * inv1ma;
				const v2f d0 = C0 - ac0[p], d1 = C1 - ac1[p], d2 = C2 - ac2[p];
				v2f dL_dalpha = __builtin_elementwise_fma(d2, dp2[p], __builtin_elementwise_fma(d1, dp1[p], d0 * dp0[p]));
				v2f dV = {0.f, 0.f};
				if (AUX) {
					dV = V - acD[p];
					dL_dalpha = __builtin_elementwise_fma(dV, dpD[p], dL_dalpha);
				}
				const v2f n0 = __builtin_elementwise_fma(alpha, d0, ac0[p]);
				const v2f n1 = __builtin_elementwise_fma(alpha, d1, ac1[p]);
				const v2f n2 = __builtin_elementwise_fma(alpha, d2, ac2[p]);
				dL_dalpha = __builtin_elementwise_fma(dL_dalpha, Tn, tfb[p] * inv1ma);
				const v2f dla = {hit0 ? dL_dalpha.x : 0.f, hit1 ? dL_dalpha.y : 0.f};
				const v2f dch = alpha * Tn;
				T[p] = Tn;
				ac0[p] = n0;
				ac1[p] = n1;
				ac2[p] = n2;
				if (AUX) {
					acD[p] = __builtin_elementwise_fma(alpha, dV, acD[p]);
					acc[9] = __builtin_elementwise_fma(dch, dpD[p], acc[9]);
				}
				acc[6] = __builtin_elementwise_fma(dch, dp0[p], acc[6]);
				acc[7] = __builtin_elementwise_fma(dch, dp1[p], acc[7]);
				acc[8] = __builtin_elementwise_fma(dch, dp2[p], acc[8]);
				acc[5] = __builtin_elementwise_fma(G, dla, acc[5]);
				const v2f f = (OP * dla) * G;
				const v2f fdx = f * dx, fdy = f * dy;
				acc[0] += fdx;
				acc[1] += fdy;
				acc[2] = __builtin_elementwise_fma(fdx, dx, acc[2]);
				acc[3] = __builtin_elementwise_fma(fdx, dy, acc[3]);
				acc[4] = __builtin_elementwise_fma(fdy, dy, acc[4]);
			}
			if (any) {
				GSR_TILE_STAT(st_reductions++;)
				float v[GSR_BWD_NV];
#pragma unroll
				for (int i = 0; i < GSR_BWD_NV; i++) v[i] = gsr_add_halves(acc[i]);
#pragma unroll
				for (int i = 0; i < 8; i++) red_w[i] = v[i];
				float col[8];
#pragma unroll
				for (int k = 0; k < 8; k++) col[k] = red_r[red_step * k];
				if constexpr (AUX) {
					__builtin_amdgcn_sched_barrier(0);
					const float t9 = gsr_wave_sum_to_lane63(v[8]);
					const float t10 = gsr_wave_sum_to_lane63(gsr_add_halves(acc[9]));
					__builtin_amdgcn_sched_barrier(0);
					const float tcol = ((col[0] + col[1]) + (col[2] + col[3])) + ((col[4] + col[5]) + (col[6] + col[7]));
					const float t8 = gsr_sum8(tcol);
					const float other = gsr_dpp_mov<0x128, 0xF, 0xF, true>(t8);
					const float r01 = k01 * __builtin_fmaf(-2.0f, (out_index == 0 ? CA.x : CC.x) * t8, CB.x * other);
					const uint32_t slot = __builtin_amdgcn_readfirstlane(__float_as_uint(R4.w));
					float* out = reinterpret_cast<float*>(slots + slot);
					const float r = out_index < 2 ? r01 : out_scale * t8;
					if ((lane & 7) == 0) out[out_index] = r;
					if (lane == 63) {
						out[8] = t9;
						out[9] = t10;
						slot_valid[slot] = 1;
					}
				} else {
					const float tcol = ((col[0] + col[1]) + (col[2] + col[3])) + ((col[4] + col[5]) + (col[6] + col[7]));
					pend_w[npend * 128] = tcol;
					pend_w[npend * 128 + 64] = v[8];
					pend_j |= (uint32_t)j << (8 * npend);
					npend++;
				}
			}
			if (!AUX && (npend == GSR_BWD_FLUSH || (npend != 0 && j == cnt - 1))) {
				__builtin_amdgcn_wave_barrier();
				const float4 q0 = *reinterpret_cast<const float4*>(pend_r), q1 = *reinterpret_cast<const float4*>(pend_r + 4);
				const uint32_t jf = (pend_j >> (8 * f_inst)) & 0xFFu;
				const float* const rj = reinterpret_cast<const float*>(&rec[0][jf]);
				const float ca = rj[4 * 64], cb = rj[4 * 64 + 2], cc = rj[8 * 64];
				const uint32_t slot = __float_as_uint(rj[16 * 64 + 3]);
				asm volatile("" ::"v"(q0.x), "v"(q1.x), "v"(ca), "v"(cb), "v"(cc), "v"(slot));
				const float t = ((q0.x + q0.y) + (q0.z + q0.w)) + ((q1.x + q1.y) + (q1.z + q1.w));
				const float t9 = gsr_sum8(t);
				const float other = gsr_dpp_mov<0xB1, 0xF, 0xF, true>(t);
				const float r01 = f_k01 * __builtin_fmaf(-2.0f, (f_val == 0 ? ca : cc) * t, cb * other);
				const float r = f_val < 2 ? r01 : f_scale * t;
				if (f_inst < npend) {
					if (f_word) reinterpret_cast<float*>(slots + slot)[lane < 32 ? f_val : 8] = lane < 32 ? r : t9;
					if (lane >= 32 && f_val == 0) slot_valid[slot] = 1;
				}
				npend = 0;
				pend_j = 0u;
				__builtin_amdgcn_wave_barrier();
			}
		}
		__builtin_amdgcn_wave_barrier();
	}
	GSR_TILE_CLOCK_STOP(gsr_backward_tile_clock, slot_id, lane, st_staged | (st_pairs << 20) | (st_pairs_hit << 42), st_reductions | (st_lanes_hit << 24));
}

void gsr_launch_render_backward(int W, int H, GsrImage img, const uint32_t* point_list, const GsrSplat* splat, const float4* checkpoints,
                                const uint32_t* slot_base, const float* bg, const float* dL_dpix, GsrGradSlot* slots,
                                uint8_t* slot_valid, bool cull, hipStream_t s, hipEvent_t t_start, hipEvent_t t_stop, const GsrAuxBlend* aux)
{
	const int gx = gsr_grid_x(W), gy = gsr_grid_y(H);
	const int ntiles = gx * gy;
	const int nslots = ntiles + (int)gsr_tile_order_max_segments(ntiles);
	const int nwg = (nslots + GSR_WAVES_PER_WG - 1) / GSR_WAVES_PER_WG;
	gsr_variant(false, aux ? GSR_AUX_DEPTH : 0, false, [&](auto, auto AUX, auto) {
		gsr_launch(gsr_render_backward_wave_kernel<AUX() != 0>, dim3(nwg), dim3(64 * GSR_WAVES_PER_WG), 0, s, t_start, t_stop, W, H, gx, nslots,
		           img.ranges, point_list, splat, checkpoints, img.final_C, slot_base, bg, img.final_T, img.n_contrib, img.tile_max_contrib,
		           img.tile_order, dL_dpix, slots, slot_valid, cull ? 1 : 0, aux ? *aux : GsrAuxBlend{});
	});
}
```

gaussian-splatting_cc-comments_amd/csrc/render_forward.hip:

```cpp
#include "render_common.h"

#ifndef GSR_FWD_DONE_STRIDE
#define GSR_FWD_DONE_STRIDE 16
#endif
#ifndef GSR_FWD_AUX_WAVES
#define GSR_FWD_AUX_WAVES 5
#endif

GSR_TILE_CLOCK_BUFFER(gsr_forward_tile_clock, gsr_debug_tile_clock_forward)

template <bool AUX>
__global__ void __launch_bounds__(64 * GSR_WAVES_PER_WG) __attribute__((amdgpu_waves_per_eu(AUX ? GSR_FWD_AUX_WAVES : 6, AUX ? GSR_FWD_AUX_WAVES : 6)))
gsr_render_forward_wave_kernel(
	int W, int H, int gx, int nslots, const uint2* __restrict__ ranges, const uint32_t* __restrict__ point_list,
	const GsrSplat* __restrict__ splat, float4* __restrict__ checkpoints, float* __restrict__ final_C, const float* __restrict__ bg, float* __restrict__ final_T,
	uint32_t* __restrict__ n_contrib, uint32_t* __restrict__ tile_max_contrib, const uint32_t* __restrict__ tile_order,
	float* __restrict__ out_color, int cull, GsrAuxBlend aux)
{
	__shared__ float4 s_rec[GSR_WAVES_PER_WG][3][64];
	const int wave = threadIdx.x >> 6, lane = threadIdx.x & 63;
	const int slot_id = blockIdx.x * GSR_WAVES_PER_WG + wave;
	if (slot_id >= nslots) return;
	GSR_TILE_CLOCK_START();
	const uint32_t entry = __builtin_amdgcn_readfirstlane(tile_order ? tile_order[slot_id] : (uint32_t)slot_id);
	if (entry == 0xFFFFFFFFu) return;
	const int tile = (int)(entry & 0x0FFFFFFFu);
	const int only = (int)(entry >> 28);
	float4(*rec)[64] = s_rec[wave];

	const int tx = tile % gx, ty = tile / gx;
	const int px = tx * GSR_TILE_X + (lane & 15);
	const int py0 = ty * GSR_TILE_Y + (lane >> 4);
	float pfx = (float)px;
	asm volatile("" : "+v"(pfx));
	const float x0f = (float)(tx * GSR_TILE_X), y0f = (float)(ty * GSR_TILE_Y);

	const uint2 range = ranges[tile];
	const int n = (int)(range.y - range.x);
	const uint32_t* plist = point_list + range.x;
	const bool heavy = n >= 2 * GSR_CKPT_STRIDE;
	bool walked_deep = false;

	float Tout[GSR_PIX_PER_LANE], C0[GSR_PIX_PER_LANE], C1[GSR_PIX_PER_LANE], C2[GSR_PIX_PER_LANE];
	float Dacc[GSR_PIX_PER_LANE];
	float pfy[GSR_PIX_PER_LANE];
	uint32_t last[GSR_PIX_PER_LANE];
	unsigned long long alive[GSR_PIX_PER_LANE];
#pragma unroll
	for (int k = 0; k < GSR_PIX_PER_LANE; k++) {
		const int py = py0 + 4 * k;
		pfy[k] = (float)py;
		asm volatile("" : "+v"(pfy[k]));
		Tout[k] = 1.0f;
		alive[k] = (only == 0 || only == k + 1) ? __builtin_amdgcn_ballot_w64(px < W && py < H) : 0ull;
		C0[k] = C1[k] = C2[k] = 0.f;
		if (AUX) Dacc[k] = 0.f;
		last[k] = 0u;
	}

	GSR_TILE_STAT(unsigned long long st_staged = 0ull; unsigned long long st_bands = 0ull; unsigned long long st_hits = 0ull;)
	float4 ra = make_float4(0, 0, 0, 0), rb = ra, rc = ra;
	if (lane < n) {
		const uint32_t id = plist[lane];
		const float4* p = reinterpret_cast<const float4*>(splat + id);
		ra = p[0]; rb = p[1]; rc = p[2];
	}
	uint32_t id_next = (64 + lane < n) ? plist[64 + lane] : 0u;

	for (int base = 0; base < n; base += 64) {
		if ((alive[0] | alive[1] | alive[2] | alive[3]) == 0ull) break;
		if (heavy && base != 0 && (base & (GSR_CKPT_STRIDE - 1)) == 0) {
			walked_deep = true;
			float4* ck = checkpoints + ((size_t)(range.x + (uint32_t)base) / GSR_CKPT_STRIDE) * 256 + lane;
#pragma unroll
			for (int k = 0; k < GSR_PIX_PER_LANE; k++)
				if (only == 0 || only == k + 1) ck[64 * k] = make_float4(Tout[k], C0[k], C1[k], C2[k]);
			if (AUX) {
				float* ckd = aux.ckpt_depth + ((size_t)(range.x + (uint32_t)base) / GSR_CKPT_STRIDE) * 256 + lane;
#pragma unroll
				for (int k = 0; k < GSR_PIX_PER_LANE; k++)
					if (only == 0 || only == k + 1) ckd[64 * k] = Dacc[k];
			}
		}
		const uint32_t bands = (base + lane < n) ? (cull ? gsr_tile_band_mask(ra.x, ra.y, ra.z, ra.w, rb.x, rb.y, x0f, y0f) : 0xFu) : 0u;
		const bool keep = bands != 0u;
		const unsigned long long mask = __builtin_amdgcn_ballot_w64(keep);
		const int cnt = __popcll(mask);
		GSR_TILE_STAT(st_staged += (unsigned long long)cnt;)
		if (keep) {
			const int pos = gsr_mbcnt(mask);
			rec[0][pos] = make_float4(ra.x, ra.y, -0.5f * ra.z, ra.w);
			rec[1][pos] = make_float4(-0.5f * rb.x, rb.y, rc.x, rc.y);
			rec[2][pos] = make_float4(rc.z, __uint_as_float((uint32_t)(base + lane + 1)), __uint_as_float(bands), AUX ? rc.w : 0.f);
		}
		if (base + 64 + lane < n) {
			const float4* p = reinterpret_cast<const float4*>(splat + id_next);
			ra = p[0]; rb = p[1]; rc = p[2];
		}
		id_next = (base + 128 + lane < n) ? plist[base + 128 + lane] : 0u;
		__builtin_amdgcn_wave_barrier();

		for (int j0 = 0; j0 < cnt; j0 += GSR_FWD_DONE_STRIDE) {
		const uint32_t open_bands = __builtin_amdgcn_readfirstlane((alive[0] ? 1u : 0u) | (alive[1] ? 2u : 0u) | (alive[2] ? 4u : 0u) | (alive[3] ? 8u : 0u));
		if (open_bands == 0u) break;
		const int j1 = min(cnt, j0 + GSR_FWD_DONE_STRIDE);
		for (int j = j0; j < j1; j++) {
			const float4 A = rec[0][j];
			const float4 B = rec[1][j];
			const float4 Cc = rec[2][j];
			const uint32_t contributor = __float_as_uint(Cc.y);
			uint32_t bands = __builtin_amdgcn_readfirstlane(__float_as_uint(Cc.z)) & open_bands;
			asm volatile("" : "+s"(bands));
			const float dx = A.x - pfx;
			const float ax2 = __fmul_rn(__fmul_rn(A.z, dx), dx), bdx = __fmul_rn(A.w, dx);
#pragma unroll
			for (int k = 0; k < GSR_PIX_PER_LANE; k++) {
				if (!(bands & (1u << k))) continue;
				const float dy = A.y - pfy[k];
				const float power = gsr_pair_power_halved(ax2, bdx, B.x, dy);
				const float alpha = fminf(0.99f, B.y * __expf(power));
				const float test_T = __fmul_rn(Tout[k], __fsub_rn(1.0f, alpha));
				const unsigned long long live = __builtin_amdgcn_ballot_w64(!(power > 0.0f)) & __builtin_amdgcn_ballot_w64(!(alpha < 1.0f / 255.0f));
				const unsigned long long passm = live & alive[k] & __builtin_amdgcn_ballot_w64(!(test_T < 0.0001f));
				GSR_TILE_STAT(st_bands++; st_hits += passm ? 1ull : 0ull;)
				alive[k] = (alive[k] & ~live) | passm;
				const bool pass = __builtin_amdgcn_inverse_ballot_w64(passm);
				const float w = pass ? alpha * Tout[k] : 0.0f;
				C0[k] = __builtin_fmaf(B.z, w, C0[k]);
				C1[k] = __builtin_fmaf(B.w, w, C1[k]);
				C2[k] = __builtin_fmaf(Cc.x, w, C2[k]);
				if (AUX) Dacc[k] = __builtin_fmaf(Cc.w, w, Dacc[k]);
				Tout[k] = pass ? test_T : Tout[k];
				last[k] = pass ? contributor : last[k];
			}
		}
		}
		__builtin_amdgcn_wave_barrier();
	}

	const float bg0 = bg[0], bg1 = bg[1], bg2 = bg[2];
	const size_t plane = (size_t)H * W;
	uint32_t m = 0u;
#pragma unroll
	for (int k = 0; k < GSR_PIX_PER_LANE; k++) {
		const int py = py0 + 4 * k;
		if (px < W && py < H && (only == 0 || only == k + 1)) {
			const uint32_t pix_id = (uint32_t)(W * py + px);
			final_T[pix_id] = Tout[k];
			n_contrib[pix_id] = last[k];
			out_color[pix_id] = C0[k] + Tout[k] * bg0;
			out_color[plane + pix_id] = C1[k] + Tout[k] * bg1;
			out_color[2 * plane + pix_id] = C2[k] + Tout[k] * bg2;
			if (walked_deep) { final_C[pix_id] = C0[k]; final_C[plane + pix_id] = C1[k]; final_C[2 * plane + pix_id] = C2[k]; }
			if (AUX) {
				aux.out_depth[pix_id] = Dacc[k];
				aux.out_alpha[pix_id] = 1.0f - Tout[k];
				if (walked_deep) aux.final_D[pix_id] = Dacc[k];
			}
			m = max(m, last[k]);
		}
	}
#pragma unroll
	for (int off = 32; off > 0; off >>= 1) m = max(m, (uint32_t)__shfl_down(m, off, 64));
	if (lane == 0) {
		if (only) atomicMax(&tile_max_contrib[tile], m);
		else tile_max_contrib[tile] = m;
	}
	GSR_TILE_CLOCK_STOP(gsr_forward_tile_clock, slot_id, lane, (unsigned long long)entry,
	                    (st_staged & 0xFFFFFull) | ((st_bands & 0x3FFFFFull) << 20) | ((st_hits & 0x3FFFFFull) << 42));
}

void gsr_launch_render_forward(int W, int H, GsrImage img, const uint32_t* point_list, const GsrSplat* splat, float4* checkpoints,
                               const float* bg, float* out_color, bool ordered, bool cull, hipStream_t s, const GsrAuxBlend* aux)
{
	const int gx = gsr_grid_x(W), gy = gsr_grid_y(H);
	const int ntiles = gx * gy;
	const int nslots = ntiles + (ordered ? 3 * (int)gsr_tile_order_max_split(ntiles) : 0);
	const int nwg = (nslots + GSR_WAVES_PER_WG - 1) / GSR_WAVES_PER_WG;
	gsr_variant(false, aux ? GSR_AUX_DEPTH : 0, false, [&](auto, auto AUX, auto) {
		gsr_launch(gsr_render_forward_wave_kernel<AUX() != 0>, dim3(nwg), dim3(64 * GSR_WAVES_PER_WG), 0, s, nullptr, nullptr, W, H, gx, nslots,
		           img.ranges, point_list, splat, checkpoints, img.final_C, bg, img.final_T, img.n_contrib, img.tile_max_contrib,
		           ordered ? img.tile_order : nullptr, out_color, cull ? 1 : 0, aux ? *aux : GsrAuxBlend{});
	});
}
```

Measured before the change: 1008 it/s.

## Emit per-slot dispatch records and prefetch next LDS splat record in render loops

The tile-order kernel now also writes a uint4 record per dispatch slot (entry, range start, walk length, segment length) into the binning buffer. Forward and backward render kernels read that one record instead of chasing tile_order, then ranges and tile_max_contrib. Both kernels also software-prefetch the next shared-memory splat record in the inner blend loop, and the backward kernel gets an optional early-id path. This cuts dependent global loads at wave start and hides LDS latency, at the cost of extra binning memory and higher register pressure.

```diff
diff --git a/gaussian-splatting_cc-comments_amd/csrc/api.hip b/gaussian-splatting_cc-comments_amd/csrc/api.hip
--- a/gaussian-splatting_cc-comments_amd/csrc/api.hip
+++ b/gaussian-splatting_cc-comments_amd/csrc/api.hip
@@ -196,12 +196,15 @@
 	o->n_contrib = off;        off = gsr_align_up(off + N * 4);
 	o->ranges = off;           off = gsr_align_up(off + T * 8);
 	o->tile_max_contrib = off; off = gsr_align_up(off + T * 4);
-	{
-		const size_t extra_f = 3 * (size_t)gsr_tile_order_max_split((int)T), extra_b = gsr_tile_order_max_segments((int)T);
-		o->tile_order = off;   off = gsr_align_up(off + (T + (extra_f > extra_b ? extra_f : extra_b) + 1) * 4);
-	}
+	o->tile_order = off;       off = gsr_align_up(off + (gsr_dispatch_records((int)T) + 1) * 4);
 	o->total = off;
 	return GSR_OK;
+}
+
+static size_t gsr_dispatch_offset(size_t end, int W, int H, size_t* at)
+{
+	*at = end;
+	return gsr_align_up(end + gsr_dispatch_records(gsr_grid_x(W) * gsr_grid_y(H)) * sizeof(uint4));
 }
 
 extern "C" int gsr_binning_layout_of(int P, int64_t R, int W, int H, gsr_binning_layout* o)
@@ -219,6 +222,8 @@
 		o->sort_table = off; off = gsr_align_up(off + (a > b ? a : b));
 	}
 	o->checkpoints = off;    off = gsr_align_up(off + gsr_checkpoint_records(R) * 256 * sizeof(float4));
+	size_t at;
+	off = gsr_dispatch_offset(off, W, H, &at);
 	o->total = off;
 	o->tile_key_bytes = (size_t)gsr_tile_key_bytes(gsr_grid_x(W) * gsr_grid_y(H), n);
 	o->column_pairs = gsr_tilebin_applies(W, H) ? 1 : 0;
@@ -240,6 +245,15 @@
 	gsr_binning_layout l;
 	return gsr_binning_layout_of(P, R, W, H, &l) == GSR_OK ? l.total : 0;
 }
+extern "C" int gsr_debug_dispatch_records(int P, int64_t R, int W, int H, size_t* offset, size_t* count)
+{
+	gsr_binning_layout l;
+	if (!offset || !count || gsr_binning_layout_of(P, R, W, H, &l) != GSR_OK) return gsr_fail(GSR_ERR_INVALID_ARGUMENT, "gsr_debug_dispatch_records: bad arguments");
+	gsr_dispatch_offset(gsr_align_up(l.checkpoints + gsr_checkpoint_records(R) * 256 * sizeof(float4)), W, H, offset);
+	*count = gsr_dispatch_records(gsr_grid_x(W) * gsr_grid_y(H));
+	return GSR_OK;
+}
+
 extern "C" size_t gsr_backward_scratch_bytes(int P, int64_t R)
 {
 	(void)P;
@@ -345,6 +359,9 @@
 	bn.tile_keys_alt = (uint32_t*)(b + l.tile_keys_alt);
 	bn.sort_table = (void*)(b + l.sort_table);
 	bn.checkpoints = (float4*)(b + l.checkpoints);
+	size_t at;
+	gsr_dispatch_offset(gsr_align_up(l.checkpoints + gsr_checkpoint_records(R) * 256 * sizeof(float4)), W, H, &at);
+	bn.dispatch = (uint4*)(b + at);
 	return bn;
 }
 
@@ -748,13 +765,13 @@
 	}
 	if (R > 0) {
 		GsrProfScope p(s, "tile_order");
-		gsr_launch_tile_order(im, ntiles, false, R, !(debug & GSR_DEBUG_NO_SPLIT), s, col_pairs);
+		gsr_launch_tile_order(im, b.dispatch, ntiles, false, R, !(debug & GSR_DEBUG_NO_SPLIT), s, col_pairs);
 	}
 	if ((rc = gsr_stage_done(s, debug, "tile_order"))) return rc;
 	{
 		GsrProfScope p(s, "render_forward");
 		GsrAuxBlend x;
-		gsr_launch_render_forward(width, height, im, b.point_list, g.splat, b.checkpoints, background, out_color, R > 0, !(debug & GSR_DEBUG_NO_CULL), s,
+		gsr_launch_render_forward(width, height, im, b.dispatch, b.point_list, g.splat, b.checkpoints, background, out_color, R > 0, !(debug & GSR_DEBUG_NO_CULL), s,
 		                          gsr_aux_view(aux, R, width, height, &x));
 	}
 	return gsr_stage_done(s, debug, "render_forward");
@@ -821,7 +838,7 @@
 	GsrBinning b = gsr_binning_view(a.binning, a.P, a.num_rendered, a.width, a.height);
 	{
 		GsrProfScope p(s, "tile_order");
-		gsr_launch_tile_order(im, gsr_grid_x(a.width) * gsr_grid_y(a.height), true, a.num_rendered, !(a.debug & GSR_DEBUG_NO_SPLIT), s);
+		gsr_launch_tile_order(im, b.dispatch, gsr_grid_x(a.width) * gsr_grid_y(a.height), true, a.num_rendered, !(a.debug & GSR_DEBUG_NO_SPLIT), s);
 	}
 	if ((rc = gsr_stage_done(s, a.debug, "tile_order"))) return rc;
 	{
@@ -829,7 +846,7 @@
 		const bool own = gsr_prof_kernel_events(s, "render_backward", &t0, &t1);
 		GsrProfScope p(s, own ? nullptr : "render_backward");
 		GsrAuxBlend x;
-		gsr_launch_render_backward(a.width, a.height, im, b.point_list, g.splat, b.checkpoints, g.slot_base, a.background, a.dL_dpix,
+		gsr_launch_render_backward(a.width, a.height, im, b.dispatch, b.point_list, g.splat, b.checkpoints, g.slot_base, a.background, a.dL_dpix,
 		                           (GsrGradSlot*)a.scratch, (uint8_t*)b.tile_keys_alt, !(a.debug & GSR_DEBUG_NO_CULL), s, t0, t1,
 		                           gsr_aux_view(aux, a.num_rendered, a.width, a.height, &x));
 	}
diff --git a/gaussian-splatting_cc-comments_amd/csrc/binning.hip b/gaussian-splatting_cc-comments_amd/csrc/binning.hip
--- a/gaussian-splatting_cc-comments_amd/csrc/binning.hip
+++ b/gaussian-splatting_cc-comments_amd/csrc/binning.hip
@@ -187,15 +187,20 @@
 
 #define GSR_ORDER_BINS 1024
 #define GSR_ORDER_PER_THREAD 9
-__device__ __forceinline__ uint32_t gsr_tile_work(const uint2* ranges, const uint32_t* tile_max_contrib, uint32_t t)
+__device__ __forceinline__ uint32_t gsr_tile_walk(const uint2* ranges, const uint32_t* tile_max_contrib, uint32_t t, uint32_t* first)
+{
+	const uint2 r = ranges[t];
+	uint32_t walk = r.y - r.x;
+	if (tile_max_contrib) walk = min(walk, tile_max_contrib[t]);
+	*first = r.x;
+	return walk;
+}
+__device__ __forceinline__ uint32_t gsr_tile_work(const uint32_t* work_key, uint32_t walk, uint32_t t)
 {
 #ifdef GSR_TILE_CLOCK
-	if (!ranges) return tile_max_contrib[t];
+	if (work_key) return work_key[t];
 #endif
-	const uint2 r = ranges[t];
-	uint32_t work = r.y - r.x;
-	if (tile_max_contrib) work = min(work, tile_max_contrib[t]);
-	return work;
+	return walk;
 }
 __device__ __forceinline__ uint32_t gsr_tile_work_bin(uint32_t work)
 {
@@ -208,6 +213,11 @@
 	const uint32_t nblk = (work + GSR_CKPT_STRIDE - 1) / GSR_CKPT_STRIDE;
 	const uint32_t m = (nblk + GSR_CKPT_MAX_SEGMENTS - 1) / GSR_CKPT_MAX_SEGMENTS * coarse;
 	return (nblk + m - 1) / m;
+}
+__device__ __forceinline__ uint32_t gsr_tile_segment_length(uint32_t work, uint32_t coarse)
+{
+	const uint32_t nblk = (work + GSR_CKPT_STRIDE - 1) / GSR_CKPT_STRIDE;
+	return (nblk + GSR_CKPT_MAX_SEGMENTS - 1) / GSR_CKPT_MAX_SEGMENTS * coarse * GSR_CKPT_STRIDE;
 }
 
 #ifdef GSR_TILE_CLOCK
@@ -220,7 +230,7 @@
 __global__ void __launch_bounds__(1024) gsr_tile_order_kernel(const uint2* ranges, const uint32_t* __restrict__ tile_max_contrib,
                                                               uint32_t ntiles, uint32_t* __restrict__ order, uint32_t split_min, uint32_t max_split,
                                                               uint32_t* tile_max_contrib_out, uint32_t seg_budget, int allow_cut,
-                                                              uint2* ranges_fix)
+                                                              uint2* ranges_fix, uint4* __restrict__ records, const uint32_t* __restrict__ work_key)
 {
 	__shared__ uint32_t bin[GSR_ORDER_BINS];
 	__shared__ uint32_t wsum[1024 / 64];
@@ -228,12 +238,13 @@
 	if (threadIdx.x == 0) { s_nsplit = 0u; s_seg_cursor = 0u; s_total = 0u; }
 	if (threadIdx.x < 4) s_seg_items[threadIdx.x] = 0u;
 	bin[threadIdx.x] = 0;
-	uint32_t b0[GSR_ORDER_PER_THREAD], w0[GSR_ORDER_PER_THREAD];
+	uint32_t b0[GSR_ORDER_PER_THREAD], w0[GSR_ORDER_PER_THREAD], x0[GSR_ORDER_PER_THREAD];
 #pragma unroll
 	for (int j = 0; j < GSR_ORDER_PER_THREAD; j++) {
 		const uint32_t t = j * 1024 + threadIdx.x;
-		w0[j] = t < ntiles ? gsr_tile_work(ranges, tile_max_contrib, t) : 0u;
-		b0[j] = t < ntiles ? gsr_tile_work_bin(w0[j]) : 0xffffffffu;
+		x0[j] = 0u;
+		w0[j] = t < ntiles ? gsr_tile_walk(ranges, tile_max_contrib, t, &x0[j]) : 0u;
+		b0[j] = t < ntiles ? gsr_tile_work_bin(gsr_tile_work(work_key, w0[j], t)) : 0xffffffffu;
 		if (ranges_fix && t < ntiles && w0[j] == 0u) ranges_fix[t] = make_uint2(0u, 0u);
 	}
 	if (ranges_fix)
@@ -252,7 +263,7 @@
 		};
 #pragma unroll
 		for (int j = 0; j < GSR_ORDER_PER_THREAD; j++) count(w0[j]);
-		for (uint32_t t = 1024 * GSR_ORDER_PER_THREAD + threadIdx.x; t < ntiles; t += 1024) count(gsr_tile_work(ranges, tile_max_contrib, t));
+		for (uint32_t t = 1024 * GSR_ORDER_PER_THREAD + threadIdx.x; t < ntiles; t += 1024) { uint32_t x; count(gsr_tile_walk(ranges, tile_max_contrib, t, &x)); }
 #pragma unroll
 		for (int f = 0; f < 4; f++)
 			if (my_items[f]) atomicAdd(&s_seg_items[f], my_items[f]);
@@ -266,8 +277,9 @@
 #pragma unroll
 		for (int j = 0; j < GSR_ORDER_PER_THREAD; j++) {
 			const uint32_t t = base + j * 1024 + threadIdx.x;
-			const uint32_t w = t < ntiles ? gsr_tile_work(ranges, tile_max_contrib, t) : 0u;
-			b[j] = t < ntiles ? gsr_tile_work_bin(w) : 0xffffffffu;
+			uint32_t x;
+			const uint32_t w = t < ntiles ? gsr_tile_walk(ranges, tile_max_contrib, t, &x) : 0u;
+			b[j] = t < ntiles ? gsr_tile_work_bin(gsr_tile_work(work_key, w, t)) : 0xffffffffu;
 			my_work += w;
 		}
 #pragma unroll
@@ -300,62 +312,74 @@
 		}
 	if (seg_budget && threadIdx.x == 0) order[ntiles + seg_budget] = coarse;
 	const uint32_t nsplit = s_nsplit;
-	auto place = [&](uint32_t q, uint32_t t) {
+	auto place = [&](uint32_t q, uint32_t t, uint32_t first, uint32_t walk) {
+		auto put = [&](uint32_t e, uint32_t entry, uint32_t seglen) {
+			order[e] = entry;
+			if (records) records[e] = make_uint4(entry, first, walk, seglen);
+		};
 		if (q < nheavy) {
-			const uint32_t ns = gsr_tile_segments(gsr_tile_work(ranges, tile_max_contrib, t), coarse);
+			const uint32_t ns = gsr_tile_segments(walk, coarse), len = gsr_tile_segment_length(walk, coarse);
 			const uint32_t at = atomicAdd(&s_seg_cursor, ns);
-			for (uint32_t k = 0; k < ns; k++) order[at + k] = t | ((k + 1u) << 28);
+			for (uint32_t k = 0; k < ns; k++) put(at + k, t | ((k + 1u) << 28), len);
 		} else if (nheavy) {
-			order[front + (q - nheavy)] = t;
+			put(front + (q - nheavy), t, 0u);
 		} else if (q < nsplit) {
 #pragma unroll
-			for (uint32_t k = 0; k < 4; k++) order[4 * q + k] = t | ((k + 1u) << 28);
+			for (uint32_t k = 0; k < 4; k++) put(4 * q + k, t | ((k + 1u) << 28), 0u);
 			tile_max_contrib_out[t] = 0u;
 		} else {
-			order[3 * nsplit + q] = t;
-		}
+			put(3 * nsplit + q, t, 0u);
+		}
+	};
+	auto unused = [&](uint32_t e) {
+		order[e] = 0xFFFFFFFFu;
+		if (records) records[e] = make_uint4(0xFFFFFFFFu, 0u, 0u, 0u);
 	};
 	if (max_split)
-		for (uint32_t e = ntiles + 3 * nsplit + threadIdx.x; e < ntiles + 3 * max_split; e += 1024) order[e] = 0xFFFFFFFFu;
+		for (uint32_t e = ntiles + 3 * nsplit + threadIdx.x; e < ntiles + 3 * max_split; e += 1024) unused(e);
 	if (seg_budget)
-		for (uint32_t e = ntiles + (front - nheavy) + threadIdx.x; e < ntiles + seg_budget; e += 1024) order[e] = 0xFFFFFFFFu;
+		for (uint32_t e = ntiles + (front - nheavy) + threadIdx.x; e < ntiles + seg_budget; e += 1024) unused(e);
 #pragma unroll
 	for (int j = 0; j < GSR_ORDER_PER_THREAD; j++)
-		if (b0[j] != 0xffffffffu) place(atomicAdd(&bin[b0[j]], 1u), j * 1024 + threadIdx.x);
+		if (b0[j] != 0xffffffffu) place(atomicAdd(&bin[b0[j]], 1u), j * 1024 + threadIdx.x, x0[j], w0[j]);
 	for (uint32_t base = 1024 * GSR_ORDER_PER_THREAD; base < ntiles; base += 1024 * GSR_ORDER_PER_THREAD) {
-		uint32_t b[GSR_ORDER_PER_THREAD];
+		uint32_t b[GSR_ORDER_PER_THREAD], w[GSR_ORDER_PER_THREAD], x[GSR_ORDER_PER_THREAD];
 #pragma unroll
 		for (int j = 0; j < GSR_ORDER_PER_THREAD; j++) {
 			const uint32_t t = base + j * 1024 + threadIdx.x;
-			b[j] = t < ntiles ? gsr_tile_work_bin(gsr_tile_work(ranges, tile_max_contrib, t)) : 0xffffffffu;
+			x[j] = 0u;
+			w[j] = t < ntiles ? gsr_tile_walk(ranges, tile_max_contrib, t, &x[j]) : 0u;
+			b[j] = t < ntiles ? gsr_tile_work_bin(gsr_tile_work(work_key, w[j], t)) : 0xffffffffu;
 		}
 #pragma unroll
 		for (int j = 0; j < GSR_ORDER_PER_THREAD; j++)
-			if (b[j] != 0xffffffffu) place(atomicAdd(&bin[b[j]], 1u), base + j * 1024 + threadIdx.x);
+			if (b[j] != 0xffffffffu) place(atomicAdd(&bin[b[j]], 1u), base + j * 1024 + threadIdx.x, x[j], w[j]);
 	}
 }
 
 uint32_t gsr_tile_order_max_segments(int ntiles) { return (uint32_t)(ntiles < 64 ? 0 : (ntiles / 2 < 4096 ? ntiles / 2 : 4096)); }
 uint32_t gsr_tile_order_max_split(int ntiles) { return (uint32_t)(ntiles < 64 ? 0 : (ntiles / 4 < 2048 ? ntiles / 4 : 2048)); }
-
-void gsr_launch_tile_order(GsrImage img, int ntiles, bool backward, int64_t num_rendered, bool split, hipStream_t s, bool normalise_empty)
-{
-	const uint32_t* key = backward ? img.tile_max_contrib : (const uint32_t*)nullptr;
-	const uint2* ranges = img.ranges;
+size_t gsr_dispatch_records(int ntiles)
+{
+	const size_t extra_f = 3 * (size_t)gsr_tile_order_max_split(ntiles), extra_b = gsr_tile_order_max_segments(ntiles);
+	return (size_t)ntiles + (extra_f > extra_b ? extra_f : extra_b);
+}
+
+void gsr_launch_tile_order(GsrImage img, uint4* records, int ntiles, bool backward, int64_t num_rendered, bool split, hipStream_t s, bool normalise_empty)
+{
+	const uint32_t* work_key = nullptr;
 #ifdef GSR_TILE_CLOCK
-	if (backward && g_debug_backward_key) { key = g_debug_backward_key; ranges = nullptr; }
-	if (!backward && g_debug_forward_key) { key = g_debug_forward_key; ranges = nullptr; split = false; }
+	if (backward && g_debug_backward_key) work_key = g_debug_backward_key;
+	if (!backward && g_debug_forward_key) { work_key = g_debug_forward_key; split = false; }
 #endif
 	(void)num_rendered;
 	const uint32_t max_split = backward ? 0u : gsr_tile_order_max_split(ntiles);
 	const uint32_t split_min = (!backward && split && max_split) ? (uint32_t)GSR_SPLIT_MIN_LIST : 0u;
 	const uint32_t seg_budget = backward ? gsr_tile_order_max_segments(ntiles) : 0u;
-	int allow_cut = split ? 1 : 0;
-#ifdef GSR_TILE_CLOCK
-	if (!ranges) allow_cut = 0;
-#endif
-	hipLaunchKernelGGL(gsr_tile_order_kernel, dim3(1), dim3(1024), 0, s, ranges, key, (uint32_t)ntiles, img.tile_order, split_min, max_split,
-	                   img.tile_max_contrib, seg_budget, allow_cut, (normalise_empty && !backward) ? img.ranges : (uint2*)nullptr);
+	const int allow_cut = (split && !work_key) ? 1 : 0;
+	hipLaunchKernelGGL(gsr_tile_order_kernel, dim3(1), dim3(1024), 0, s, (const uint2*)img.ranges, backward ? (const uint32_t*)img.tile_max_contrib : (const uint32_t*)nullptr,
+	                   (uint32_t)ntiles, img.tile_order, split_min, max_split, img.tile_max_contrib, seg_budget, allow_cut,
+	                   (normalise_empty && !backward) ? img.ranges : (uint2*)nullptr, records, work_key);
 }
 
 void gsr_launch_tile_ranges(const void* tile_keys, int key_bytes, int64_t R, uint2* ranges, int ntiles, uint32_t* valid, hipStream_t s)
diff --git a/gaussian-splatting_cc-comments_amd/csrc/gsr_internal.h b/gaussian-splatting_cc-comments_amd/csrc/gsr_internal.h
--- a/gaussian-splatting_cc-comments_amd/csrc/gsr_internal.h
+++ b/gaussian-splatting_cc-comments_amd/csrc/gsr_internal.h
@@ -65,6 +65,7 @@
 	uint32_t* tile_keys_alt;
 	void* sort_table;
 	float4* checkpoints;
+	uint4* dispatch;
 };
 
 struct GsrAuxBlend {
@@ -149,9 +150,10 @@
 void gsr_launch_sorted_block_sums(GsrGeometry g, int P, int result_in_alt, hipStream_t s);
 void gsr_launch_duplicate_keys(GsrGeometry g, int P, int W, void* keys, int key_bytes, uint32_t* vals, uint32_t* clear, size_t clear_words, hipStream_t s);
 void gsr_launch_tile_ranges(const void* tile_keys, int key_bytes, int64_t R, uint2* ranges, int ntiles, uint32_t* valid, hipStream_t s);
-void gsr_launch_tile_order(GsrImage img, int ntiles, bool backward, int64_t num_rendered, bool split, hipStream_t s, bool normalise_empty = false);
+void gsr_launch_tile_order(GsrImage img, uint4* records, int ntiles, bool backward, int64_t num_rendered, bool split, hipStream_t s, bool normalise_empty = false);
 uint32_t gsr_tile_order_max_split(int ntiles);
 uint32_t gsr_tile_order_max_segments(int ntiles);
+size_t gsr_dispatch_records(int ntiles);
 
 bool gsr_tilebin_applies(int W, int H);
 size_t gsr_tilebin_col_clear_words(size_t P);
@@ -183,11 +185,11 @@
 void gsr_launch_depth_bucket_sort(GsrGeometry g, int P, uint4* seg, hipStream_t s);
 int gsr_tile_key_bytes(int ntiles, size_t num_rendered);
 
-void gsr_launch_render_forward(int W, int H, GsrImage img, const uint32_t* point_list, const GsrSplat* splat, float4* checkpoints,
+void gsr_launch_render_forward(int W, int H, GsrImage img, const uint4* dispatch, const uint32_t* point_list, const GsrSplat* splat, float4* checkpoints,
                                const float* bg, float* out_color, bool ordered, bool cull, hipStream_t s,
                                const GsrAuxBlend* aux);
 
-void gsr_launch_render_backward(int W, int H, GsrImage img, const uint32_t* point_list, const GsrSplat* splat, const float4* checkpoints,
+void gsr_launch_render_backward(int W, int H, GsrImage img, const uint4* dispatch, const uint32_t* point_list, const GsrSplat* splat, const float4* checkpoints,
                                 const uint32_t* slot_base, const float* bg, const float* dL_dpix, GsrGradSlot* slots,
                                 uint8_t* slot_valid, bool cull, hipStream_t s, hipEvent_t t_start, hipEvent_t t_stop,
                                 const GsrAuxBlend* aux);
diff --git a/gaussian-splatting_cc-comments_amd/csrc/render_backward.hip b/gaussian-splatting_cc-comments_amd/csrc/render_backward.hip
--- a/gaussian-splatting_cc-comments_amd/csrc/render_backward.hip
+++ b/gaussian-splatting_cc-comments_amd/csrc/render_backward.hip
@@ -1,5 +1,11 @@
 #include "render_common.h"
 
+#ifndef GSR_BWD_EARLY_IDS
+#define GSR_BWD_EARLY_IDS 1
+#endif
+#ifndef GSR_BWD_PREFETCH
+#define GSR_BWD_PREFETCH 1
+#endif
 #define GSR_BWD_NV 9
 #define GSR_BWD_FLUSH 4
 typedef float v2f __attribute__((ext_vector_type(2)));
@@ -15,10 +21,10 @@
 
 template <bool AUX>
 __global__ void __launch_bounds__(64 * GSR_WAVES_PER_WG) __attribute__((amdgpu_waves_per_eu(4, 4))) gsr_render_backward_wave_kernel(
-	int W, int H, int gx, int nslots, const uint2* __restrict__ ranges, const uint32_t* __restrict__ point_list,
+	int W, int H, int gx, int nslots, const uint32_t* __restrict__ point_list,
 	const GsrSplat* __restrict__ splat, const float4* __restrict__ checkpoints, const float* __restrict__ final_C, const uint32_t* __restrict__ slot_base, const float* __restrict__ bg,
-	const float* __restrict__ final_Ts, const uint32_t* __restrict__ n_contrib, const uint32_t* __restrict__ tile_max_contrib,
-	const uint32_t* __restrict__ tile_order, const float* __restrict__ dL_dpixels, GsrGradSlot* __restrict__ slots,
+	const float* __restrict__ final_Ts, const uint32_t* __restrict__ n_contrib,
+	const uint4* __restrict__ dispatch, const float* __restrict__ dL_dpixels, GsrGradSlot* __restrict__ slots,
 	uint8_t* __restrict__ slot_valid, int cull, GsrAuxBlend aux)
 {
 	__shared__ float4 s_rec[GSR_WAVES_PER_WG][AUX ? 6 : 5][64];
@@ -30,7 +36,9 @@
 	if (slot_id >= nslots) return;
 	GSR_TILE_CLOCK_START();
 	GSR_TILE_STAT(unsigned long long st_staged = 0; unsigned long long st_pairs = 0; unsigned long long st_pairs_hit = 0; unsigned long long st_reductions = 0; unsigned long long st_lanes_hit = 0;)
-	const uint32_t entry = __builtin_amdgcn_readfirstlane(tile_order[slot_id]);
+	const uint4 drec = dispatch[__builtin_amdgcn_readfirstlane(slot_id)];
+	const uint32_t entry = __builtin_amdgcn_readfirstlane(drec.x);
+	asm volatile("" ::"s"(drec.y), "s"(drec.z), "s"(drec.w));
 	if (entry == 0xFFFFFFFFu) return;
 	const int tile = (int)(entry & 0x0FFFFFFFu);
 	const int seg1 = (int)(entry >> 28);
@@ -43,17 +51,20 @@
 	const v2f pfx2 = {(float)px, (float)px};
 	const float x0f = (float)(tx * GSR_TILE_X), y0f = (float)(ty * GSR_TILE_Y);
 
-	const uint2 range = ranges[tile];
-	const int n = (int)min(range.y - range.x, tile_max_contrib[tile]);
+	const uint32_t range_x = __builtin_amdgcn_readfirstlane(drec.y);
+	const int n = (int)__builtin_amdgcn_readfirstlane(drec.z);
 	int seg_a = 0, top = n;
 	if (seg1) {
-		const int coarse = (int)__builtin_amdgcn_readfirstlane(tile_order[nslots]);
-		const int nblk = (n + GSR_CKPT_STRIDE - 1) / GSR_CKPT_STRIDE, m = (nblk + GSR_CKPT_MAX_SEGMENTS - 1) / GSR_CKPT_MAX_SEGMENTS * coarse;
-		seg_a = (seg1 - 1) * m * GSR_CKPT_STRIDE;
-		top = min(n, seg1 * m * GSR_CKPT_STRIDE);
+		const int len = (int)__builtin_amdgcn_readfirstlane(drec.w);
+		seg_a = (seg1 - 1) * len;
+		top = min(n, seg1 * len);
 	}
 	const int nw = top - seg_a;
-	const uint32_t* plist = point_list + range.x;
+	const uint32_t* plist = point_list + range_x;
+#if GSR_BWD_EARLY_IDS
+	uint32_t id_first = (lane < nw) ? plist[top - 1 - lane] : 0u;
+	uint32_t id_next = (64 + lane < nw) ? plist[top - 1 - (64 + lane)] : 0u;
+#endif
 	const size_t plane = (size_t)H * W;
 	const float bg0 = bg[0], bg1 = bg[1], bg2 = bg[2];
 	const float ddelx_dx = 0.5f * W, ddely_dy = 0.5f * H;
@@ -92,7 +103,7 @@
 		if (AUX) acD[p] = v2f{0.f, 0.f};
 	}
 	if (top < n) {
-		const float4* ck = checkpoints + ((size_t)(range.x + (uint32_t)top) / GSR_CKPT_STRIDE) * 256 + lane;
+		const float4* ck = checkpoints + ((size_t)(range_x + (uint32_t)top) / GSR_CKPT_STRIDE) * 256 + lane;
 #pragma unroll
 		for (int k = 0; k < GSR_PIX_PER_LANE; k++) {
 			const int py = py0 + 4 * k;
@@ -105,7 +116,7 @@
 				ac0[k >> 1][k & 1] = (final_C[pix_id] - c.y) * inv;
 				ac1[k >> 1][k & 1] = (final_C[plane + pix_id] - c.z) * inv;
 				ac2[k >> 1][k & 1] = (final_C[2 * plane + pix_id] - c.w) * inv;
-				if (AUX) acD[k >> 1][k & 1] = (aux.final_D[pix_id] - aux.ckpt_depth[((size_t)(range.x + (uint32_t)top) / GSR_CKPT_STRIDE) * 256 + lane + 64 * k]) * inv;
+				if (AUX) acD[k >> 1][k & 1] = (aux.final_D[pix_id] - aux.ckpt_depth[((size_t)(range_x + (uint32_t)top) / GSR_CKPT_STRIDE) * 256 + lane + 64 * k]) * inv;
 			}
 		}
 	}
@@ -120,6 +131,13 @@
 
 	float4 ra = make_float4(0, 0, 0, 0), rb = ra, rc = ra;
 	uint32_t sbase = 0u;
+#if GSR_BWD_EARLY_IDS
+	if (lane < nw) {
+		const float4* p = reinterpret_cast<const float4*>(splat + id_first);
+		ra = p[0]; rb = p[1]; rc = p[2];
+		sbase = slot_base[id_first];
+	}
+#else
 	if (lane < nw) {
 		const uint32_t id = plist[top - 1 - lane];
 		const float4* p = reinterpret_cast<const float4*>(splat + id);
@@ -127,6 +145,7 @@
 		sbase = slot_base[id];
 	}
 	uint32_t id_next = (64 + lane < nw) ? plist[top - 1 - (64 + lane)] : 0u;
+#endif
 	const int out_index = lane >> 3;
 	float* const red_w = s_red[wave] + lane * 9;
 	const float* const red_r = s_red[wave] + (lane & 7) * 9 + (lane >> 3);
@@ -168,9 +187,20 @@
 		id_next = (base + 128 + lane < nw) ? plist[top - 1 - (base + 128 + lane)] : 0u;
 		__builtin_amdgcn_wave_barrier();
 
+		constexpr bool PREFETCH = GSR_BWD_PREFETCH && !AUX;
+		float4 nR0, nR1, nR2;
+		if constexpr (PREFETCH) { nR0 = rec[0][0]; nR1 = rec[1][0]; nR2 = rec[2][0]; }
 #pragma clang loop unroll(disable)
 		for (int j = 0; j < cnt; j++) {
-			const float4 R0 = rec[0][j], R1 = rec[1][j], R2 = rec[2][j], R3 = rec[3][j], R4 = rec[4][j];
+			float4 R0, R1, R2;
+			if constexpr (PREFETCH) {
+				R0 = nR0; R1 = nR1; R2 = nR2;
+				const int jn = min(j + 1, cnt - 1);
+				nR0 = rec[0][jn]; nR1 = rec[1][jn]; nR2 = rec[2][jn];
+			} else {
+				R0 = rec[0][j]; R1 = rec[1][j]; R2 = rec[2][j];
+			}
+			const float4 R3 = rec[3][j], R4 = rec[4][j];
 			const int contributor = __builtin_amdgcn_readfirstlane(__float_as_int(R4.z));
 			const uint32_t bands = __builtin_amdgcn_readfirstlane(recb[j]);
 			const v2f X = {R0.x, R0.y}, Y = {R0.z, R0.w}, CA = {R1.x, R1.y}, CB = {R1.z, R1.w}, CC = {R2.x, R2.y}, OP = {R2.z, R2.w};
@@ -301,7 +331,7 @@
 	GSR_TILE_CLOCK_STOP(gsr_backward_tile_clock, slot_id, lane, st_staged | (st_pairs << 20) | (st_pairs_hit << 42), st_reductions | (st_lanes_hit << 24));
 }
 
-void gsr_launch_render_backward(int W, int H, GsrImage img, const uint32_t* point_list, const GsrSplat* splat, const float4* checkpoints,
+void gsr_launch_render_backward(int W, int H, GsrImage img, const uint4* dispatch, const uint32_t* point_list, const GsrSplat* splat, const float4* checkpoints,
                                 const uint32_t* slot_base, const float* bg, const float* dL_dpix, GsrGradSlot* slots,
                                 uint8_t* slot_valid, bool cull, hipStream_t s, hipEvent_t t_start, hipEvent_t t_stop, const GsrAuxBlend* aux)
 {
@@ -311,7 +341,7 @@
 	const int nwg = (nslots + GSR_WAVES_PER_WG - 1) / GSR_WAVES_PER_WG;
 	gsr_variant(false, aux ? GSR_AUX_DEPTH : 0, false, [&](auto, auto AUX, auto) {
 		gsr_launch(gsr_render_backward_wave_kernel<AUX() != 0>, dim3(nwg), dim3(64 * GSR_WAVES_PER_WG), 0, s, t_start, t_stop, W, H, gx, nslots,
-		           img.ranges, point_list, splat, checkpoints, img.final_C, slot_base, bg, img.final_T, img.n_contrib, img.tile_max_contrib,
-		           img.tile_order, dL_dpix, slots, slot_valid, cull ? 1 : 0, aux ? *aux : GsrAuxBlend{});
+		           point_list, splat, checkpoints, img.final_C, slot_base, bg, img.final_T, img.n_contrib,
+		           dispatch, dL_dpix, slots, slot_valid, cull ? 1 : 0, aux ? *aux : GsrAuxBlend{});
 	});
 }
diff --git a/gaussian-splatting_cc-comments_amd/csrc/render_forward.hip b/gaussian-splatting_cc-comments_amd/csrc/render_forward.hip
--- a/gaussian-splatting_cc-comments_amd/csrc/render_forward.hip
+++ b/gaussian-splatting_cc-comments_amd/csrc/render_forward.hip
@@ -1,5 +1,8 @@
 #include "render_common.h"
 
+#ifndef GSR_FWD_PREFETCH
+#define GSR_FWD_PREFETCH 1
+#endif
 #ifndef GSR_FWD_DONE_STRIDE
 #define GSR_FWD_DONE_STRIDE 16
 #endif
@@ -14,7 +17,7 @@
 gsr_render_forward_wave_kernel(
 	int W, int H, int gx, int nslots, const uint2* __restrict__ ranges, const uint32_t* __restrict__ point_list,
 	const GsrSplat* __restrict__ splat, float4* __restrict__ checkpoints, float* __restrict__ final_C, const float* __restrict__ bg, float* __restrict__ final_T,
-	uint32_t* __restrict__ n_contrib, uint32_t* __restrict__ tile_max_contrib, const uint32_t* __restrict__ tile_order,
+	uint32_t* __restrict__ n_contrib, uint32_t* __restrict__ tile_max_contrib, const uint4* __restrict__ dispatch,
 	float* __restrict__ out_color, int cull, GsrAuxBlend aux)
 {
 	__shared__ float4 s_rec[GSR_WAVES_PER_WG][3][64];
@@ -22,7 +25,9 @@
 	const int slot_id = blockIdx.x * GSR_WAVES_PER_WG + wave;
 	if (slot_id >= nslots) return;
 	GSR_TILE_CLOCK_START();
-	const uint32_t entry = __builtin_amdgcn_readfirstlane(tile_order ? tile_order[slot_id] : (uint32_t)slot_id);
+	uint4 drec = make_uint4((uint32_t)slot_id, 0u, 0u, 0u);
+	if (dispatch) drec = dispatch[__builtin_amdgcn_readfirstlane(slot_id)];
+	const uint32_t entry = __builtin_amdgcn_readfirstlane(drec.x);
 	if (entry == 0xFFFFFFFFu) return;
 	const int tile = (int)(entry & 0x0FFFFFFFu);
 	const int only = (int)(entry >> 28);
@@ -35,7 +40,8 @@
 	asm volatile("" : "+v"(pfx));
 	const float x0f = (float)(tx * GSR_TILE_X), y0f = (float)(ty * GSR_TILE_Y);
 
-	const uint2 range = ranges[tile];
+	uint2 range = make_uint2(__builtin_amdgcn_readfirstlane(drec.y), __builtin_amdgcn_readfirstlane(drec.y + drec.z));
+	if (!dispatch) range = ranges[tile];
 	const int n = (int)(range.y - range.x);
 	const uint32_t* plist = point_list + range.x;
 	const bool heavy = n >= 2 * GSR_CKPT_STRIDE;
@@ -100,14 +106,22 @@
 		id_next = (base + 128 + lane < n) ? plist[base + 128 + lane] : 0u;
 		__builtin_amdgcn_wave_barrier();
 
+		constexpr bool PREFETCH = GSR_FWD_PREFETCH && !AUX;
+		float4 nA, nB, nC;
+		if constexpr (PREFETCH) { nA = rec[0][0]; nB = rec[1][0]; nC = rec[2][0]; }
 		for (int j0 = 0; j0 < cnt; j0 += GSR_FWD_DONE_STRIDE) {
 		const uint32_t open_bands = __builtin_amdgcn_readfirstlane((alive[0] ? 1u : 0u) | (alive[1] ? 2u : 0u) | (alive[2] ? 4u : 0u) | (alive[3] ? 8u : 0u));
 		if (open_bands == 0u) break;
 		const int j1 = min(cnt, j0 + GSR_FWD_DONE_STRIDE);
 		for (int j = j0; j < j1; j++) {
-			const float4 A = rec[0][j];
-			const float4 B = rec[1][j];
-			const float4 Cc = rec[2][j];
+			float4 A, B, Cc;
+			if constexpr (PREFETCH) {
+				A = nA; B = nB; Cc = nC;
+				const int jn = min(j + 1, cnt - 1);
+				nA = rec[0][jn]; nB = rec[1][jn]; nC = rec[2][jn];
+			} else {
+				A = rec[0][j]; B = rec[1][j]; Cc = rec[2][j];
+			}
 			const uint32_t contributor = __float_as_uint(Cc.y);
 			uint32_t bands = __builtin_amdgcn_readfirstlane(__float_as_uint(Cc.z)) & open_bands;
 			asm volatile("" : "+s"(bands));
@@ -170,7 +184,7 @@
 	                    (st_staged & 0xFFFFFull) | ((st_bands & 0x3FFFFFull) << 20) | ((st_hits & 0x3FFFFFull) << 42));
 }
 
-void gsr_launch_render_forward(int W, int H, GsrImage img, const uint32_t* point_list, const GsrSplat* splat, float4* checkpoints,
+void gsr_launch_render_forward(int W, int H, GsrImage img, const uint4* dispatch, const uint32_t* point_list, const GsrSplat* splat, float4* checkpoints,
                                const float* bg, float* out_color, bool ordered, bool cull, hipStream_t s, const GsrAuxBlend* aux)
 {
 	const int gx = gsr_grid_x(W), gy = gsr_grid_y(H);
@@ -180,6 +194,6 @@
 	gsr_variant(false, aux ? GSR_AUX_DEPTH : 0, false, [&](auto, auto AUX, auto) {
 		gsr_launch(gsr_render_forward_wave_kernel<AUX() != 0>, dim3(nwg), dim3(64 * GSR_WAVES_PER_WG), 0, s, nullptr, nullptr, W, H, gx, nslots,
 		           img.ranges, point_list, splat, checkpoints, img.final_C, bg, img.final_T, img.n_contrib, img.tile_max_contrib,
-		           ordered ? img.tile_order : nullptr, out_color, cull ? 1 : 0, aux ? *aux : GsrAuxBlend{});
+		           ordered ? dispatch : nullptr, out_color, cull ? 1 : 0, aux ? *aux : GsrAuxBlend{});
 	});
 }
```

New measurement: 970.3 it/s. 0.963x the previous value.
